# MAdrid1011/transplat

Hardware: AMD Instinct MI355X
Metric: novel views/sec at 256x256, 2 ctx views; PSNR parity vs reference (higher is better)
Workload: dtype fp32 (bf16x3 dense, >= TF32) + bf16x3 attention + fp32 raster; 1 GPU; e2e TranSplat test_step: 1 scene(s) x (2 ctx -> 3 tgt) 256x256; dense mode bf16x3 (split-bf16 products, fp32 accumulation; >= TF32), window-attention mode bf16x3; parallelism=scene-shard x1

## Files before the change

include/transplat_hip.h:

```cpp
#ifndef TRANSPLAT_HIP_H
#define TRANSPLAT_HIP_H

#include <stddef.h>
#include <stdint.h>

#ifdef __cplusplus
extern "C" {
#endif

#define TSPLAT_OK 0
#define TSPLAT_EINVAL (-1)
#define TSPLAT_EHIP (-2)

int tsplat_version(void);

int tsplat_set_debug(int32_t on);

int tsplat_prof_enable(int32_t kernel_id);
int tsplat_prof_read(double* total_ms, int32_t* launches);

typedef struct tsplat_raster_desc {
    int32_t num_gaussians;
    int32_t num_views;
    int32_t views_per_scene;
    int32_t height;
    int32_t width;
    int32_t sh_coeffs;
    int32_t sh_degree;
    int32_t capacity;
} tsplat_raster_desc;

size_t tsplat_raster_workspace_bytes(int32_t num_gaussians, int32_t num_views, int32_t height,
                                     int32_t width, int32_t capacity);

size_t tsplat_raster_num_rendered_offset(int32_t num_gaussians, int32_t num_views, int32_t height,
                                         int32_t width);

int tsplat_raster_fwd(const tsplat_raster_desc* desc,
                      const float* means, const float* cov, const float* shs,
                      const float* opacity, const float* viewmat, const float* projmat,
                      const float* campos, const float* tanfov, const float* bg,
                      const float* scene_scale,
                      float* out_color, int32_t* out_radii,
                      void* workspace, int32_t* status, void* stream);

int tsplat_raster_depth_fwd(const tsplat_raster_desc* desc,
                            const float* means, const float* cov, const float* shs,
                            const float* opacity, const float* viewmat, const float* projmat,
                            const float* campos, const float* tanfov, const float* bg,
                            const float* scene_scale, const float* near, const float* far,
                            int32_t depth_mode,
                            float* out_color, float* out_depth, float* out_alpha,
                            int32_t* out_radii, void* workspace, int32_t* status, void* stream);

size_t tsplat_raster_bwd_workspace_bytes(int32_t num_gaussians, int32_t num_views);

int tsplat_raster_bwd(const tsplat_raster_desc* desc,
                      const float* means, const float* cov, const float* shs,
                      const float* opacity, const float* viewmat, const float* projmat,
                      const float* campos, const float* tanfov, const float* bg,
                      const float* scene_scale,
                      const float* out_color, const float* grad_color, const int32_t* radii,
                      void* fwd_workspace, void* bwd_workspace,
                      float* grad_means, float* grad_cov, float* grad_shs, float* grad_opacity,
                      void* stream);

int tsplat_raster_depth_bwd(const tsplat_raster_desc* desc,
                            const float* means, const float* cov, const float* shs,
                            const float* opacity, const float* viewmat, const float* projmat,
                            const float* campos, const float* tanfov, const float* bg,
                            const float* scene_scale, const float* near, const float* far,
                            int32_t depth_mode,
                            const float* out_color, const float* out_depth, const float* out_alpha,
                            const float* grad_color, const float* grad_depth,
                            const float* grad_alpha, const int32_t* radii,
                            void* fwd_workspace, void* bwd_workspace,
                            float* grad_means, float* grad_cov, float* grad_shs, float* grad_opacity,
                            void* stream);


int tsplat_depth_softmax_fwd(const float* logits, const float* disp, float* coarse, float* pdf_max, int32_t n,
                             int32_t depths, int32_t hw, void* stream);

int tsplat_depth_tail_fwd(const float* fullres, const float* head, const float* near, const float* far, float* depth,
                          float* density, int32_t batch, int32_t views, int32_t hw, void* stream);

int tsplat_raster_cameras(const float* extrinsics, const float* intrinsics, const float* near, const float* far,
                          const float* bg, int32_t bg_per_view, int32_t scale_invariant, int32_t num_views,
                          float* viewmat, float* projmat, float* campos, float* tanfov, float* bg_out, float* scale,
                          void* stream);


int tsplat_uv_coarse_fwd(const float* feat, const float* cams, const float* disp, float* out,
                         int32_t batch, int32_t height, int32_t width, int32_t channels,
                         int32_t depths, void* stream);

int tsplat_uv_cross_fwd(const float* value, const float* key, const float* cams,
                        const float* disp, const float* offsets, const float* logits, float* out,
                        int32_t batch, int32_t height, int32_t width, int32_t channels,
                        int32_t depths, int32_t points, void* stream);

int tsplat_uv_cross_table_fwd(const float* table, const float* cams, const float* disp, const float* offsets,
                              const float* logits, float* out, int32_t batch, int32_t height, int32_t width,
                              int32_t channels, int32_t depths, int32_t points, void* stream);

size_t tsplat_uv_cross_pack_bytes(int32_t batch, int32_t height, int32_t width);
int tsplat_uv_cross_pack_fwd(const float* value, void* packed, int32_t batch, int32_t height, int32_t width,
                             int32_t channels, void* stream);
int tsplat_uv_cross_fused_fwd(const void* packed, const float* key, const float* cams, const float* disp,
                              const float* offsets, const float* logits, float* out, int32_t batch,
                              int32_t height, int32_t width, int32_t channels, int32_t depths, int32_t points,
                              void* stream);
int tsplat_uv_cross_pack_ld_fwd(const float* value, int32_t ld_value, void* packed, int32_t batch, int32_t height,
                                int32_t width, int32_t channels, void* stream);
int tsplat_uv_cross_fused_ld_fwd(const void* packed, const float* key, const float* cams, const float* disp,
                                 const float* offsets, int32_t ld_offsets, const float* logits, int32_t ld_logits,
                                 float* out, int32_t batch, int32_t height, int32_t width, int32_t channels,
                                 int32_t depths, int32_t points, void* stream);

int tsplat_msda_fwd(const float* value, const float* loc, const float* weights, float* out,
                    int32_t n, int32_t height, int32_t width, int32_t channels, int32_t queries,
                    int32_t points, void* stream);

int tsplat_msda_raw_fwd(const float* value, const float* ow, float* out, int32_t n, int32_t height, int32_t width,
                        int32_t channels, int32_t points, int32_t ow_stride, void* stream);

int tsplat_ms_deform_attn_fwd(const float* value, const int64_t* spatial_shapes, const int64_t* level_start_index,
                              const float* sampling_loc, const float* attn_weight, float* out, int32_t batch,
                              int32_t num_keys, int32_t num_heads, int32_t head_dim, int32_t num_levels,
                              int32_t num_queries, int32_t num_points, int32_t im2col_step, void* stream);

int tsplat_sh_rotation_fwd(const float* rotations, const double* basis, float* out, int32_t num_cameras,
                           int32_t d_sh, void* stream);

size_t tsplat_group_norm_workspace_bytes(int32_t n, int32_t c, int64_t hw, int32_t groups);
int tsplat_group_norm_fwd(const float* x, const float* pre_bias, const float* gamma, const float* beta,
                          const float* residual,
                          float* y, void* workspace, int32_t n, int32_t c, int64_t hw, int32_t groups,
                          float eps, int32_t act, void* stream);
int tsplat_group_norm_cat_res_fwd(const float* x, const float* pre_bias, const float* gamma, const float* beta,
                                  const float* residual, const float* residual2, int32_t c1, float* y,
                                  void* workspace, int32_t n, int32_t c, int64_t hw, int32_t groups, float eps,
                                  int32_t act, void* stream);
int tsplat_group_norm_bf16_fwd(const void* x, const float* pre_bias, const float* gamma, const float* beta,
                               const void* residual, void* y, void* workspace, int32_t n, int32_t c, int64_t hw,
                               int32_t groups, float eps, int32_t act, void* stream);

int tsplat_bias_act_fwd(const float* x, const float* bias, const float* residual, float* y, int32_t n, int32_t c,
                        int64_t hw, int32_t act, void* stream);

int tsplat_bias_act_nhwc_fwd(const float* x, const float* bias, const float* res1, const float* res2, float* y,
                             int64_t rows, int32_t c, int32_t act, void* stream);

int tsplat_residual_ln_fwd(const float* x, const float* y, const float* ls, const float* ln_w, const float* ln_b,
                           float ln_eps, float* x_out, float* n_out, int32_t rows, int32_t dim, void* stream);
int tsplat_layer_norm128_fwd(const void* y, int32_t y_bf16, const float* residual, const float* ln_w,
                             const float* ln_b, float ln_eps, void* out, int32_t out_bf16, int32_t rows,
                             void* stream);
int tsplat_residual_ln_bf16_fwd(const float* x, const void* y, const float* ls, const float* ln_w, const float* ln_b,
                                float ln_eps, float* x_out, void* n_out, int32_t rows, int32_t dim, void* stream);

int tsplat_gaussian_adapter_fwd(const float* raw, const float* depths, const float* densities,
                                const float* cams, const float* sh_rot, float* means, float* cov,
                                float* harmonics, float* opacities, int32_t batch, int32_t views,
                                int32_t height, int32_t width, int32_t raw_ch, int32_t d_sh,
                                float scale_min, float scale_max, float opacity_exponent,
                                int32_t gaussians_per_pixel, int32_t raw_nchw, void* stream);

size_t tsplat_win_attn_workspace_bytes(int32_t batch, int32_t height, int32_t width, int32_t key_views,
                                       int32_t splits);
int tsplat_win_attn_fwd(const float* q, const float* k, const float* v, float* out, void* workspace,
                        int32_t batch, int32_t height, int32_t width, int32_t channels,
                        int32_t key_views, int32_t splits, int32_t with_shift, void* stream);

int32_t tsplat_win_attn_split(int32_t batch, int32_t height, int32_t width, int32_t key_views, int32_t splits);
int tsplat_win_attn_partials_fwd(const float* q, const float* k, const float* v, void* workspace, int32_t batch,
                                 int32_t height, int32_t width, int32_t channels, int32_t key_views,
                                 int32_t splits, int32_t with_shift, int32_t key_batch_shift, void* stream);

int tsplat_split_kv_bf16x3(const float* k, const float* v, void* kv_x3, int64_t n, void* stream);
int tsplat_linear_f32_split_x3_fwd(const float* x1, int32_t k1, const float* w, float* out, void* kv_x3, int32_t M,
                                   int32_t N, int32_t x3_from, int32_t flags, void* stream);
int tsplat_win_attn_x3_fwd(const float* q, const void* kv_x3, float* out, void* workspace, int32_t batch,
                           int32_t height, int32_t width, int32_t channels, int32_t key_views, int32_t splits,
                           int32_t with_shift, void* stream);
int tsplat_win_attn_x3_partials_fwd(const float* q, const void* kv_x3, void* workspace, int32_t batch, int32_t height,
                                    int32_t width, int32_t channels, int32_t key_views, int32_t splits,
                                    int32_t with_shift, int32_t key_batch_shift, void* stream);

size_t tsplat_win_attn_bf16_workspace_bytes(int32_t batch, int32_t height, int32_t width, int32_t key_views,
                                            int32_t splits);
int tsplat_win_attn_bf16_fwd(const void* q, const void* k, const void* v, void* out, void* workspace,
                             int32_t batch, int32_t height, int32_t width, int32_t channels,
                             int32_t key_views, int32_t splits, int32_t with_shift, void* stream);
int tsplat_win_attn_bf16_shift_fwd(const void* q, const void* k, const void* v, void* out, void* workspace,
                                   int32_t batch, int32_t height, int32_t width, int32_t channels,
                                   int32_t key_views, int32_t splits, int32_t with_shift,
                                   int32_t key_batch_shift, void* stream);

int tsplat_linear_f32_fwd(const float* x1, int32_t k1, const float* x2, int32_t k2, const float* w,
                          const float* bias, const float* ln_gamma, const float* ln_beta, float ln_eps,
                          const float* residual, float* out, int64_t split_stride, int32_t M, int32_t N,
                          int32_t flags, void* stream);

int tsplat_linear_f32_attn_merge_fwd(const float* partials, int32_t batch, int32_t height, int32_t width,
                                     int32_t key_views, int32_t splits, int32_t with_shift, const float* w,
                                     const float* ln_gamma, const float* ln_beta, float ln_eps,
                                     const float* residual, float* out, int32_t N, int32_t flags, void* stream);

int tsplat_small_inverse(const float* in, float* out, int32_t n, int32_t dim, void* stream);

int tsplat_pack_cameras_fwd(const float* intr, const float* pose, float* cams, int32_t n, void* stream);

int tsplat_cam_gate_fwd(const float* cam, const float* w1, const float* b1, const float* w2, const float* b2,
                        const float* w3, const float* b3, const float* w4, const float* b4, float* gate,
                        int32_t views, int32_t in_features, int32_t channels, void* stream);

int tsplat_mha_f32_fwd(const float* qkv, float* out, int32_t batch, int32_t tokens, int32_t heads,
                       int32_t head_dim, float scale, void* stream);
int tsplat_mha_bias_f32_fwd(const float* qkv, const float* bias, float* out, int32_t batch, int32_t tokens,
                            int32_t heads, int32_t head_dim, float scale, void* stream);
int tsplat_mha_x3_presplit_fwd(const void* qkv_hi, const void* qkv_lo, float* out, int32_t batch, int32_t tokens,
                               int32_t heads, int32_t head_dim, float scale, void* stream);
size_t tsplat_mha_x3_workspace_bytes(int32_t batch, int32_t tokens, int32_t heads, int32_t head_dim);
int tsplat_mha_x3_fwd(const float* qkv, const float* bias, float* out, void* workspace, int32_t batch,
                      int32_t tokens, int32_t heads, int32_t head_dim, float scale, void* stream);

int tsplat_qkv_attention_cf_fwd(const float* qkv, float* out, int32_t batch, int32_t heads, int32_t views,
                                int32_t tokens_per_view, int32_t head_dim, float scale, void* stream);

int tsplat_conv2d_f32_fwd(const float* x1, int32_t c1, const float* x2, int32_t c2, const float* w_packed,
                          const float* bias, float* y, int32_t batch, int32_t height, int32_t width, int32_t c_out,
                          int32_t ksize, int32_t stride, int32_t upsample, int32_t ksplit, void* stream);

int tsplat_conv2d_f32_zsplit_fwd(const float* x1, int32_t c1, const float* x2, int32_t c2, const float* w_packed,
                                 const float* bias, float* y, int32_t batch, int32_t height, int32_t width,
                                 int32_t c_out, int32_t ksize, int32_t stride, int32_t upsample, int32_t ksplit,
                                 int32_t zsplit, float* partials, int32_t* counters, void* stream);

int tsplat_conv2d_bf16x3_fwd(const float* x1, int32_t c1, const float* x2, int32_t c2, const void* w_packed,
                             const float* bias, float* y, int32_t batch, int32_t height, int32_t width,
                             int32_t c_out, int32_t ksize, int32_t stride, int32_t upsample, int32_t ksplit,
                             int32_t zsplit, float* partials, int32_t* counters, void* stream);
int tsplat_conv1x1_bf16x3_scaled_fwd(const float* x, int32_t c_in, const float* scale, const void* w_packed,
                                     const float* bias, float* y, int32_t batch, int32_t height, int32_t width,
                                     int32_t c_out, int32_t channel_last, int32_t ksplit, int32_t zsplit,
                                     float* partials, int32_t* counters, void* stream);

size_t tsplat_wino_weight_floats(int32_t c_out, int32_t c_in);
int tsplat_wino_weight_f32(const float* weight, float* w_packed, int32_t c_out, int32_t c_in, void* stream);
int tsplat_conv3x3_wino_f32_fwd(const float* x, const float* w_packed, const float* bias, float* y, int32_t batch,
                                int32_t c_in, int32_t height, int32_t width, int32_t c_out, int32_t act,
                                void* stream);
int tsplat_conv3x3_wino_cat_f32_fwd(const float* const* srcs, const int32_t* chans, int32_t n_src,
                                    const float* w_packed, const float* bias, float* y, int32_t batch,
                                    int32_t height, int32_t width, int32_t c_out, int32_t act, void* stream);

size_t tsplat_wino_weight_bf16x3_bytes(int32_t c_out, int32_t c_in);
int tsplat_wino_weight_bf16x3(const float* weight, void* w_packed, int32_t c_out, int32_t c_in, void* stream);
int tsplat_conv3x3_wino_bf16x3_fwd(const float* x, const void* w_packed, const float* bias, float* y, int32_t batch,
                                   int32_t c_in, int32_t height, int32_t width, int32_t c_out, int32_t act,
                                   void* stream);
int tsplat_conv3x3_wino_bf16x3_cat_fwd(const float* const* srcs, const int32_t* chans, int32_t n_src,
                                       const void* w_packed, const float* bias, float* y, int32_t batch,
                                       int32_t height, int32_t width, int32_t c_out, int32_t act, void* stream);
int tsplat_conv3x3_wino_bf16x3_ex_fwd(const float* const* srcs, const int32_t* chans, int32_t n_src,
                                      const void* w_packed, const float* bias, const float* residual,
                                      const float* residual2, float* y, int32_t batch, int32_t height, int32_t width,
                                      int32_t c_out, int32_t act, int32_t relu_in, void* stream);

int32_t tsplat_conv3x3_few_form(int32_t batch, int32_t c_in, int32_t height, int32_t width, int32_t c_out);
int tsplat_conv3x3_few_bf16x3_fwd(const float* const* srcs, const int32_t* chans, int32_t n_src,
                                  const void* w_packed, const float* bias, const float* residual,
                                  const float* residual2, float* y, int32_t batch, int32_t height, int32_t width,
                                  int32_t c_out, int32_t act, int32_t relu_in, void* stream);

int tsplat_split_bf16x3(const float* x, void* out, int64_t rows, int32_t k, int32_t weight_order, void* stream);

size_t tsplat_conv2d_bf16_weight_bytes(int32_t c_out, int32_t c_in, int32_t ksize);
int tsplat_conv2d_bf16_fwd(const void* const* srcs, const int32_t* src_channels, int32_t n_src, const int32_t* src_f32,
                           const void* w_packed, const float* bias, void* y, int32_t batch, int32_t height,
                           int32_t width, int32_t c_out, int32_t ksize, int32_t upsample, int32_t act,
                           void* stream);

int tsplat_conv2d_f32_nhwc_fwd(const float* x, int32_t c_in, const float* w_packed, const float* bias,
                               const float* residual, float* y, int32_t batch, int32_t height, int32_t width,
                               int32_t c_out, int32_t ksize, int32_t relu_in, int32_t ksplit, void* stream);

int tsplat_upsample_bilinear_act_fwd(const float* x, const float* bias, float* y, int32_t n, int32_t c,
                                     int32_t height, int32_t width, int32_t scale, int32_t act, void* stream);

int tsplat_resize_bilinear_nhwc_fwd(const float* x, float* y, int32_t n, int32_t height, int32_t width, int32_t c,
                                    int32_t out_height, int32_t out_width, void* stream);

int tsplat_resize_bilinear_nchw_fwd(const float* x, float* y, int32_t planes, int32_t height, int32_t width,
                                    int32_t out_height, int32_t out_width, void* stream);

size_t tsplat_gemm_x3_pack_bytes(int32_t n, int32_t k);
int tsplat_gemm_x3_pack(const float* w, void* wp, int32_t n, int32_t k, void* stream);
int tsplat_gemm_x3_fwd(const float* x, const void* wp, const float* bias, float* out, int32_t m, int32_t n, int32_t k,
                       int32_t ksplit, int32_t act, void* stream);
int tsplat_gemm_x3_cat_fwd(const float* x1, int32_t k1, const float* x2, int32_t k2, const void* wp, const float* bias,
                           float* out, int32_t m, int32_t n, int32_t ksplit, int32_t act, void* stream);

int tsplat_residual_ln_slabs_fwd(const float* x, const float* y, int32_t nslab, const float* ls, const float* ln_w,
                                 const float* ln_b, float ln_eps, float* x_out, float* n_out, int32_t rows,
                                 int32_t dim, void* stream);
int tsplat_residual_ln_slabs_bcast_fwd(const float* x, int32_t x_rows, const float* y, int32_t nslab, const float* ls,
                                       const float* ln_w, const float* ln_b, float ln_eps, float* x_out, float* n_out,
                                       int32_t rows, int32_t dim, void* stream);

int tsplat_da_patches_fwd(const float* image, const float* mean, const float* stdv, float* out, int32_t nimg,
                          int32_t height, int32_t width, int32_t grid_h, int32_t grid_w, int32_t patch, void* stream);

int32_t tsplat_depth_norm_blocks(int32_t out_height, int32_t out_width);
int tsplat_depth_norm_fwd(const float* x, float* resized, float* partials, float* out, int32_t nimg, int32_t height,
                          int32_t width, int32_t out_height, int32_t out_width, void* stream);

size_t tsplat_ssim_workspace_bytes(int32_t n, int32_t height, int32_t width);
int tsplat_ssim_fwd(const float* gt, const float* pred, float* ssim, void* workspace, int32_t n, int32_t height,
                    int32_t width, void* stream);

int tsplat_lpips_scale_fwd(const float* gt, const float* pred, float* out, int32_t n, int32_t height, int32_t width,
                           void* stream);
int32_t tsplat_lpips_tap_blocks(int32_t channels, int32_t height, int32_t width);
size_t tsplat_lpips_workspace_bytes(int32_t n, int32_t channels, int32_t height, int32_t width);
int tsplat_lpips_tap_fwd(const float* feat, const float* lin, void* partials, float* pooled, int32_t n,
                         int32_t channels, int32_t height, int32_t width, void* stream);
int tsplat_lpips_reduce_fwd(const void* workspace, const int32_t* blocks, const int64_t* pixels, int32_t ntaps,
                            float* out, float* out_layers, int32_t n, void* stream);


int tsplat_trajectory_extrinsics(const float* initial, const float* final_, const float* t, double eps,
                                 int32_t num_pairs, int32_t num_steps, float* out, void* stream);

size_t tsplat_quantile_workspace_bytes(int32_t num_requests);
int tsplat_quantile_f32(const float* x, int64_t n, const double* q, const int32_t* positive_only,
                        int32_t num_requests, double* out, void* workspace, void* stream);

int tsplat_video_frames_fwd(const float* color, const float* depth, const double* quantiles, int32_t frames,
                            int32_t height, int32_t width, uint8_t* out, void* stream);

int tsplat_timestamp(void* buf, int32_t slot, void* stream);

#ifdef __cplusplus
}
#endif

#endif
```

transplat_amd/_lib.py:

```python
from __future__ import annotations

import ctypes
import os
from pathlib import Path

import torch

_LIB_PATH = Path(os.environ.get("TSPLAT_LIB") or Path(__file__).resolve().parent / "libtransplat_hip.so")
_lib = None


class RasterDesc(ctypes.Structure):
    _fields_ = [
        ("num_gaussians", ctypes.c_int32),
        ("num_views", ctypes.c_int32),
        ("views_per_scene", ctypes.c_int32),
        ("height", ctypes.c_int32),
        ("width", ctypes.c_int32),
        ("sh_coeffs", ctypes.c_int32),
        ("sh_degree", ctypes.c_int32),
        ("capacity", ctypes.c_int32),
    ]


_P = ctypes.c_void_p
_I32 = ctypes.c_int32

SIGNATURES = {
    "tsplat_version": (ctypes.c_int, []),
    "tsplat_set_debug": (ctypes.c_int, [_I32]),
    "tsplat_timestamp": (ctypes.c_int, [_P, _I32, _P]),
    "tsplat_prof_enable": (ctypes.c_int, [_I32]),
    "tsplat_prof_read": (ctypes.c_int, [ctypes.POINTER(ctypes.c_double), ctypes.POINTER(_I32)]),
    "tsplat_raster_workspace_bytes": (ctypes.c_size_t, [_I32, _I32, _I32, _I32, _I32]),
    "tsplat_raster_num_rendered_offset": (ctypes.c_size_t, [_I32, _I32, _I32, _I32]),
    "tsplat_raster_fwd": (
        ctypes.c_int,
        [ctypes.POINTER(RasterDesc)] + [_P] * 15,
    ),
    "tsplat_raster_depth_fwd": (
        ctypes.c_int,
        [ctypes.POINTER(RasterDesc)] + [_P] * 12 + [_I32] + [_P] * 7,
    ),
    "tsplat_raster_bwd_workspace_bytes": (ctypes.c_size_t, [_I32, _I32]),
    "tsplat_raster_bwd": (
        ctypes.c_int,
        [ctypes.POINTER(RasterDesc)] + [_P] * 20,
    ),
    "tsplat_raster_depth_bwd": (
        ctypes.c_int,
        [ctypes.POINTER(RasterDesc)] + [_P] * 12 + [_I32] + [_P] * 14,
    ),
    "tsplat_uv_coarse_fwd": (ctypes.c_int, [_P] * 4 + [_I32] * 5 + [_P]),
    "tsplat_uv_cross_fwd": (ctypes.c_int, [_P] * 7 + [_I32] * 6 + [_P]),
    "tsplat_uv_cross_table_fwd": (ctypes.c_int, [_P] * 6 + [_I32] * 6 + [_P]),
    "tsplat_uv_cross_pack_bytes": (ctypes.c_size_t, [_I32] * 3),
    "tsplat_uv_cross_pack_fwd": (ctypes.c_int, [_P, _P] + [_I32] * 4 + [_P]),
    "tsplat_uv_cross_fused_fwd": (ctypes.c_int, [_P] * 7 + [_I32] * 6 + [_P]),
    "tsplat_uv_cross_pack_ld_fwd": (ctypes.c_int, [_P, _I32, _P] + [_I32] * 4 + [_P]),
    "tsplat_uv_cross_fused_ld_fwd": (ctypes.c_int, [_P] * 5 + [_I32, _P, _I32, _P] + [_I32] * 6 + [_P]),
    "tsplat_msda_fwd": (ctypes.c_int, [_P] * 4 + [_I32] * 6 + [_P]),
    "tsplat_msda_raw_fwd": (ctypes.c_int, [_P, _P, _P] + [_I32] * 6 + [_P]),
    "tsplat_ms_deform_attn_fwd": (ctypes.c_int, [_P] * 6 + [_I32] * 8 + [_P]),
    "tsplat_win_attn_workspace_bytes": (ctypes.c_size_t, [_I32] * 5),
    "tsplat_win_attn_fwd": (ctypes.c_int, [_P] * 5 + [_I32] * 7 + [_P]),
    "tsplat_win_attn_bf16_workspace_bytes": (ctypes.c_size_t, [_I32] * 5),
    "tsplat_win_attn_bf16_fwd": (ctypes.c_int, [_P] * 5 + [_I32] * 7 + [_P]),
    "tsplat_win_attn_bf16_shift_fwd": (ctypes.c_int, [_P] * 5 + [_I32] * 8 + [_P]),
    "tsplat_group_norm_workspace_bytes": (ctypes.c_size_t, [_I32, _I32, ctypes.c_int64, _I32]),
    "tsplat_group_norm_fwd": (ctypes.c_int, [_P] * 7 + [_I32, _I32, ctypes.c_int64, _I32, ctypes.c_float, _I32, _P]),
    "tsplat_group_norm_cat_res_fwd": (ctypes.c_int, [_P] * 6 + [_I32, _P, _P, _I32, _I32, ctypes.c_int64, _I32,
                                                                ctypes.c_float, _I32, _P]),
    "tsplat_layer_norm128_fwd": (ctypes.c_int, [_P, _I32, _P, _P, _P, ctypes.c_float, _P, _I32, _I32, _P]),
    "tsplat_group_norm_bf16_fwd": (ctypes.c_int, [_P] * 7 + [_I32, _I32, ctypes.c_int64, _I32, ctypes.c_float, _I32,
                                                            _P]),
    "tsplat_sh_rotation_fwd": (ctypes.c_int, [_P] * 3 + [_I32] * 2 + [_P]),
    "tsplat_gaussian_adapter_fwd": (ctypes.c_int, [_P] * 9 + [_I32] * 6 + [ctypes.c_float] * 3 + [_I32, _I32, _P]),
    "tsplat_win_attn_split": (_I32, [_I32] * 5),
    "tsplat_depth_softmax_fwd": (ctypes.c_int, [_P] * 4 + [_I32] * 3 + [_P]),
    "tsplat_depth_tail_fwd": (ctypes.c_int, [_P] * 6 + [_I32] * 3 + [_P]),
    "tsplat_ssim_workspace_bytes": (ctypes.c_size_t, [_I32] * 3),
    "tsplat_ssim_fwd": (ctypes.c_int, [_P] * 4 + [_I32] * 3 + [_P]),
    "tsplat_lpips_scale_fwd": (ctypes.c_int, [_P] * 3 + [_I32] * 3 + [_P]),
    "tsplat_lpips_tap_blocks": (_I32, [_I32] * 3),
    "tsplat_lpips_workspace_bytes": (ctypes.c_size_t, [_I32] * 4),
    "tsplat_lpips_tap_fwd": (ctypes.c_int, [_P] * 4 + [_I32] * 4 + [_P]),
    "tsplat_lpips_reduce_fwd": (ctypes.c_int, [_P, _P, _P, _I32, _P, _P, _I32, _P]),
    "tsplat_raster_cameras": (ctypes.c_int, [_P] * 5 + [_I32] * 3 + [_P] * 7),
    "tsplat_small_inverse": (ctypes.c_int, [_P, _P, _I32, _I32, _P]),
    "tsplat_trajectory_extrinsics": (ctypes.c_int, [_P, _P, _P, ctypes.c_double, _I32, _I32, _P, _P]),
    "tsplat_quantile_workspace_bytes": (ctypes.c_size_t, [_I32]),
    "tsplat_quantile_f32": (ctypes.c_int, [_P, ctypes.c_int64, ctypes.POINTER(ctypes.c_double),
                                           ctypes.POINTER(_I32), _I32, _P, _P, _P]),
    "tsplat_video_frames_fwd": (ctypes.c_int, [_P, _P, _P, _I32, _I32, _I32, _P, _P]),
    "tsplat_pack_cameras_fwd": (ctypes.c_int, [_P, _P, _P, _I32, _P]),
    "tsplat_cam_gate_fwd": (ctypes.c_int, [_P] * 10 + [_I32] * 3 + [_P]),
    "tsplat_mha_f32_fwd": (ctypes.c_int, [_P, _P, _I32, _I32, _I32, _I32, ctypes.c_float, _P]),
    "tsplat_mha_bias_f32_fwd": (ctypes.c_int, [_P, _P, _P, _I32, _I32, _I32, _I32, ctypes.c_float, _P]),
    "tsplat_mha_x3_workspace_bytes": (ctypes.c_size_t, [_I32] * 4),
    "tsplat_mha_x3_fwd": (ctypes.c_int, [_P, _P, _P, _P, _I32, _I32, _I32, _I32, ctypes.c_float, _P]),
    "tsplat_mha_x3_presplit_fwd": (ctypes.c_int, [_P, _P, _P, _I32, _I32, _I32, _I32, ctypes.c_float, _P]),
    "tsplat_qkv_attention_cf_fwd": (ctypes.c_int, [_P, _P] + [_I32] * 5 + [ctypes.c_float, _P]),
    "tsplat_conv2d_f32_fwd": (ctypes.c_int, [_P, _I32, _P, _I32, _P, _P, _P] + [_I32] * 8 + [_P]),
    "tsplat_conv2d_f32_zsplit_fwd": (ctypes.c_int, [_P, _I32, _P, _I32, _P, _P, _P] + [_I32] * 9 + [_P, _P, _P]),
    "tsplat_conv2d_bf16x3_fwd": (ctypes.c_int, [_P, _I32, _P, _I32, _P, _P, _P] + [_I32] * 9 + [_P, _P, _P]),
    "tsplat_conv1x1_bf16x3_scaled_fwd": (ctypes.c_int, [_P, _I32, _P, _P, _P, _P] + [_I32] * 7 + [_P, _P, _P]),
    "tsplat_resize_bilinear_nhwc_fwd": (ctypes.c_int, [_P, _P] + [_I32] * 6 + [_P]),
    "tsplat_resize_bilinear_nchw_fwd": (ctypes.c_int, [_P, _P] + [_I32] * 5 + [_P]),
    "tsplat_upsample_bilinear_act_fwd": (ctypes.c_int, [_P, _P, _P] + [_I32] * 6 + [_P]),
    "tsplat_conv2d_f32_nhwc_fwd": (ctypes.c_int, [_P, _I32, _P, _P, _P, _P] + [_I32] * 7 + [_P]),
    "tsplat_residual_ln_fwd": (ctypes.c_int, [_P] * 5 + [ctypes.c_float, _P, _P, _I32, _I32, _P]),
    "tsplat_residual_ln_slabs_fwd": (ctypes.c_int, [_P, _P, _I32, _P, _P, _P, ctypes.c_float, _P, _P, _I32, _I32, _P]),
    "tsplat_gemm_x3_pack_bytes": (ctypes.c_size_t, [_I32, _I32]),
    "tsplat_gemm_x3_pack": (ctypes.c_int, [_P, _P, _I32, _I32, _P]),
    "tsplat_gemm_x3_fwd": (ctypes.c_int, [_P, _P, _P, _P, _I32, _I32, _I32, _I32, _I32, _P]),
    "tsplat_gemm_x3_cat_fwd": (ctypes.c_int, [_P, _I32, _P, _I32, _P, _P, _P] + [_I32] * 4 + [_P]),
    "tsplat_residual_ln_slabs_bcast_fwd": (ctypes.c_int, [_P, _I32, _P, _I32, _P, _P, _P, ctypes.c_float, _P, _P, _I32,
                                                          _I32, _P]),
    "tsplat_da_patches_fwd": (ctypes.c_int, [_P] * 4 + [_I32] * 6 + [_P]),
    "tsplat_depth_norm_blocks": (_I32, [_I32, _I32]),
    "tsplat_depth_norm_fwd": (ctypes.c_int, [_P] * 4 + [_I32] * 5 + [_P]),
    "tsplat_residual_ln_bf16_fwd": (ctypes.c_int, [_P] * 5 + [ctypes.c_float, _P, _P, _I32, _I32, _P]),
    "tsplat_bias_act_fwd": (ctypes.c_int, [_P] * 4 + [_I32, _I32, ctypes.c_int64, _I32, _P]),
    "tsplat_bias_act_nhwc_fwd": (ctypes.c_int, [_P, _P, _P, _P, _P, ctypes.c_int64, _I32, _I32, _P]),
    "tsplat_win_attn_partials_fwd": (ctypes.c_int, [_P] * 4 + [_I32] * 8 + [_P]),
    "tsplat_split_kv_bf16x3": (ctypes.c_int, [_P, _P, _P, ctypes.c_int64, _P]),
    "tsplat_linear_f32_split_x3_fwd": (ctypes.c_int, [_P, _I32, _P, _P, _P] + [_I32] * 4 + [_P]),
    "tsplat_win_attn_x3_fwd": (ctypes.c_int, [_P] * 4 + [_I32] * 7 + [_P]),
    "tsplat_win_attn_x3_partials_fwd": (ctypes.c_int, [_P] * 3 + [_I32] * 8 + [_P]),
    "tsplat_linear_f32_attn_merge_fwd": (ctypes.c_int, [_P] + [_I32] * 6 + [_P] * 3 + [ctypes.c_float, _P, _P, _I32,
                                                                                       _I32, _P]),
    "tsplat_linear_f32_fwd": (ctypes.c_int, [_P, _I32, _P, _I32] + [_P] * 4 + [ctypes.c_float, _P, _P, ctypes.c_int64]
                              + [_I32] * 3 + [_P]),
    "tsplat_wino_weight_floats": (ctypes.c_size_t, [_I32, _I32]),
    "tsplat_wino_weight_f32": (ctypes.c_int, [_P, _P, _I32, _I32, _P]),
    "tsplat_conv3x3_wino_f32_fwd": (ctypes.c_int, [_P, _P, _P, _P] + [_I32] * 6 + [_P]),
    "tsplat_conv3x3_wino_cat_f32_fwd": (ctypes.c_int, [_P, _P, _I32, _P, _P, _P] + [_I32] * 5 + [_P]),
    "tsplat_wino_weight_bf16x3_bytes": (ctypes.c_size_t, [_I32, _I32]),
    "tsplat_wino_weight_bf16x3": (ctypes.c_int, [_P, _P, _I32, _I32, _P]),
    "tsplat_conv3x3_wino_bf16x3_fwd": (ctypes.c_int, [_P, _P, _P, _P] + [_I32] * 6 + [_P]),
    "tsplat_conv3x3_wino_bf16x3_cat_fwd": (ctypes.c_int, [_P, _P, _I32, _P, _P, _P] + [_I32] * 5 + [_P]),
    "tsplat_conv3x3_wino_bf16x3_ex_fwd": (ctypes.c_int, [_P, _P, _I32, _P, _P, _P, _P, _P] + [_I32] * 6 + [_P]),
    "tsplat_conv3x3_few_form": (ctypes.c_int32, [_I32] * 5),
    "tsplat_conv3x3_few_bf16x3_fwd": (ctypes.c_int, [_P, _P, _I32, _P, _P, _P, _P, _P] + [_I32] * 6 + [_P]),
    "tsplat_split_bf16x3": (ctypes.c_int, [_P, _P, ctypes.c_int64, _I32, _I32, _P]),
    "tsplat_conv2d_bf16_weight_bytes": (ctypes.c_size_t, [_I32, _I32, _I32]),
    "tsplat_conv2d_bf16_fwd": (ctypes.c_int, [_P, _P, _I32, _P, _P, _P, _P] + [_I32] * 7 + [_P]),
}

ERRORS = {-1: "invalid argument", -2: "HIP launch error"}


def lib_path() -> Path:
    return _LIB_PATH


def load(build_if_missing: bool = False):
    global _lib
    if _lib is not None:
        return _lib
    if not _LIB_PATH.exists():
        if build_if_missing:
            from .build import build

            build()
        else:
            raise RuntimeError(
                f"transplat HIP library not built ({_LIB_PATH}); run `python -m transplat_amd.build`"
            )
    lib = ctypes.CDLL(str(_LIB_PATH), mode=os.RTLD_NOW | os.RTLD_GLOBAL)
    for name, (res, args) in SIGNATURES.items():
        fn = getattr(lib, name)
        fn.restype = res
        fn.argtypes = args
    if os.environ.get("TSPLAT_DEBUG", "0") == "1":
        lib.tsplat_set_debug(1)
    _lib = lib
    return lib


def debug_enabled() -> bool:
    lib = load()
    was = lib.tsplat_set_debug(1)
    lib.tsplat_set_debug(was)
    return bool(was)


ROUTE_HOOK = None


def check(status: int, what: str, route: str | None = None) -> None:
    if status != 0:
        raise RuntimeError(f"{what} failed: {ERRORS.get(status, status)}")
    if ROUTE_HOOK is not None:
        ROUTE_HOOK(what, route)


def ptr(t: torch.Tensor | None) -> int | None:
    if t is None:
        return None
    if not t.is_cuda:
        raise RuntimeError("transplat HIP ops need device tensors (no CPU path)")
    return t.data_ptr()


def stream_ptr(device: torch.device | None = None) -> int:
    return torch.cuda.current_stream(device).cuda_stream


PROF_IDS = {"raster_preprocess": 1, "raster_scan": 2, "raster_scatter": 3, "raster_render": 4,
            "uv_coarse": 5, "uv_cross": 6, "msda": 7, "win_attn": 8, "raster": 9,
            "group_norm": 10, "uv_cross_table": 11, "linear": 12, "mha": 13, "conv": 14, "wino_conv": 15,
            "gemm_x3": 16, "raster_bwd_render": 17, "raster_bwd_preprocess": 18, "raster_bwd": 19}


def prof_enable(name: str | None) -> None:
    check(load().tsplat_prof_enable(PROF_IDS[name] if name else 0), "tsplat_prof_enable")


def prof_read() -> tuple[float, int]:
    ms = ctypes.c_double(0.0)
    n = _I32(0)
    check(load().tsplat_prof_read(ctypes.byref(ms), ctypes.byref(n)), "tsplat_prof_read")
    return ms.value, n.value
```

transplat_amd/csrc/conv.hip:

```cpp
#include "common.h"
#include "mfma.h"
#include "prof.h"

namespace tsplat {
namespace conv {

constexpr int kMaxWaves = 16;

struct Args {
    const float* x1;
    const float* x2;
    const float* wp;
    const float* bias;
    const float* res;
    const float* scale;
    int cl_out;
    float* y;
    float* part;
    int* cnt;
    int zsplit;
    int c1, c2, cout, n;
    int hin, win;
    int hv, wv;
    int hout, wout;
    int npx;
};

template <bool NHWC>
__device__ __forceinline__ void tile_epilogue(const Args& p, const floatx16& acc, float* sred) {
    const int lane = threadIdx.x & 63, w = threadIdx.x >> 6, ksplit = blockDim.x >> 6;
    const int cot = blockIdx.y;
    const int hwo = p.hout * p.wout;
#pragma unroll
    for (int r = 0; r < 16; ++r) sred[(w * 16 + r) * 64 + lane] = acc[r];
    __syncthreads();
    const int tile = blockIdx.x + gridDim.x * blockIdx.y;
    if (p.zsplit > 1) {
        typedef __attribute__((address_space(1))) unsigned gu32;
        unsigned* mine = reinterpret_cast<unsigned*>(p.part + ((size_t)tile * p.zsplit + blockIdx.z) * 1024);
        for (int idx = threadIdx.x; idx < 1024; idx += blockDim.x) {
            float s = 0.f;
            for (int k = 0; k < ksplit; ++k) s += sred[(k * 16 + (idx >> 6)) * 64 + (idx & 63)];
            __hip_atomic_store((gu32*)(mine + idx), __float_as_uint(s), __ATOMIC_RELAXED, __HIP_MEMORY_SCOPE_AGENT);
        }
        asm volatile("s_waitcnt vmcnt(0)" ::: "memory");
        __syncthreads();
        int* flag = reinterpret_cast<int*>(sred + ksplit * 1024);
        if (threadIdx.x == 0) {
            const int t = __hip_atomic_fetch_add(p.cnt + tile, 1, __ATOMIC_RELEASE, __HIP_MEMORY_SCOPE_AGENT);
            const bool last = t == p.zsplit - 1;
            if (last) {
                __builtin_amdgcn_fence(__ATOMIC_ACQUIRE, "agent");
                asm volatile("s_waitcnt vmcnt(0)" ::: "memory");
                __hip_atomic_store(p.cnt + tile, 0, __ATOMIC_RELAXED, __HIP_MEMORY_SCOPE_AGENT);
            }
            *flag = last;
        }
        __syncthreads();
        if (!*flag) return;
        const float* all = p.part + (size_t)tile * p.zsplit * 1024;
        for (int idx = threadIdx.x; idx < 1024; idx += blockDim.x) {
            float s = 0.f;
            for (int z = 0; z < p.zsplit; ++z) s += all[(size_t)z * 1024 + idx];
            sred[idx] = s;
        }
        __syncthreads();
    }
    const int nsum = p.zsplit > 1 ? 1 : ksplit;
    for (int idx = threadIdx.x; idx < 1024; idx += blockDim.x) {
        int r, l;
        if (NHWC) {
            const int col = idx & 31, pl = idx >> 5;
            r = ((col >> 3) << 2) | (col & 3);
            l = ((col >> 2) & 1) * 32 + pl;
        } else {
            r = idx >> 6;
            l = idx & 63;
        }
        float s = 0.f;
        for (int k = 0; k < nsum; ++k) s += sred[(k * 16 + r) * 64 + l];
        const int co = cot * 32 + 8 * (r >> 2) + 4 * (l >> 5) + (r & 3);
        const int q = blockIdx.x * 32 + (l & 31);
        if (co >= p.cout || q >= p.npx) continue;
        if (p.bias) s += p.bias[co];
        size_t o;
        if (NHWC) {
            o = (size_t)q * p.cout + co;
        } else {
            const int qn = q / hwo, qp = q - qn * hwo;
            o = ((size_t)qn * p.cout + co) * hwo + qp;
        }
        if (p.res) s += p.res[o];
        p.y[o] = s;
    }
}

template <int KS, int S, int UP, int G, bool NHWC, bool RELU>
__global__ void __launch_bounds__(1024) conv_f32_kernel(Args p) {
    extern __shared__ float sred[];
    constexpr int T = KS * KS, PAD = KS / 2;
    constexpr int B = G * T;
    const int lane = threadIdx.x & 63, w = threadIdx.x >> 6, ksplit = blockDim.x >> 6;
    const int c = lane & 31, h = lane >> 5;
    const int cot = blockIdx.y;
    const int hwo = p.hout * p.wout, hwi = p.hin * p.win;
    const int px = blockIdx.x * 32 + c;
    const int pxc = min(px, p.npx - 1);
    const int nb = pxc / hwo, pix = pxc - nb * hwo;
    const int oy = pix / p.wout, ox = pix - oy * p.wout;
    const int cp_all = (p.c1 + p.c2) >> 1, cp1 = p.c1 >> 1;

    int off[T];
    unsigned vmask = 0;
#pragma unroll
    for (int t = 0; t < T; ++t) {
        const int ky = t / KS, kx = t - ky * KS;
        const int iy = oy * S + ky - PAD, ix = ox * S + kx - PAD;
        const bool v = px < p.npx && iy >= 0 && iy < p.hv && ix >= 0 && ix < p.wv;
        if (NHWC)
            off[t] = v ? (nb * hwi + iy * p.win + ix) * p.c1 : 0;
        else
            off[t] = v ? (UP ? (iy >> 1) * p.win + (ix >> 1) : iy * p.win + ix) : 0;
        vmask |= (unsigned)v << t;
    }
    const size_t wtap = (size_t)cp_all * 64;
    const float* wbase = p.wp + (size_t)cot * T * wtap + lane;
    auto chan = [&](int cp) -> const float* {
        if (NHWC) return p.x1 + 2 * cp + h;
        return cp < cp1 ? p.x1 + ((size_t)nb * p.c1 + 2 * cp + h) * hwi
                        : p.x2 + ((size_t)nb * p.c2 + 2 * (cp - cp1) + h) * hwi;
    };
    const int gw = blockIdx.z * ksplit + w, gstride = ksplit * p.zsplit;
    const int ncp = cp_all > gw ? (cp_all - gw + gstride - 1) / gstride : 0;
    const int nbatch = (ncp + G - 1) / G;
    auto load = [&](int bi, float* a, float* b) {
#pragma unroll
        for (int g = 0; g < G; ++g) {
            const int i = bi * G + g;
            const bool ok = i < ncp;
            const int cp = gw + min(i, ncp - 1) * gstride;
            const float* src = chan(cp);
            const float* wq = wbase + (size_t)cp * 64;
#pragma unroll
            for (int t = 0; t < T; ++t) {
                const float av = wq[t * wtap];
                const float bv = RELU ? fmaxf(src[off[t]], 0.f) : src[off[t]];
                const unsigned ma = ok ? ~0u : 0u;
                const unsigned mb = (ok && ((vmask >> t) & 1)) ? ~0u : 0u;
                a[g * T + t] = __uint_as_float(__float_as_uint(av) & ma);
                b[g * T + t] = __uint_as_float(__float_as_uint(bv) & mb);
            }
        }
    };

    floatx16 acc;
#pragma unroll
    for (int r = 0; r < 16; ++r) acc[r] = 0.f;
    if constexpr (KS == 3) {
        const int nb = G == 4 ? min(nbatch, 1) : nbatch;
#pragma unroll 1
        for (int bi = 0; bi < nb; ++bi) {
            float ca[B], cb[B];
            load(bi, ca, cb);
            __builtin_amdgcn_sched_barrier(0);
#pragma unroll
            for (int k = 0; k < B; ++k) acc = __builtin_amdgcn_mfma_f32_32x32x2f32(ca[k], cb[k], acc, 0, 0, 0);
        }
    } else {
        float ca[B], cb[B], na[B], nbv[B];
        if (nbatch > 0) load(0, ca, cb);
        __builtin_amdgcn_sched_barrier(0);
#pragma unroll 1
        for (int bi = 0; bi < nbatch; ++bi) {
            const bool more = bi + 1 < nbatch;
            if (more) load(bi + 1, na, nbv);
            __builtin_amdgcn_sched_barrier(0);
#pragma unroll
            for (int k = 0; k < B; ++k) acc = __builtin_amdgcn_mfma_f32_32x32x2f32(ca[k], cb[k], acc, 0, 0, 0);
            if (more) {
#pragma unroll
                for (int k = 0; k < B; ++k) {
                    ca[k] = na[k];
                    cb[k] = nbv[k];
                }
            }
        }
    }

    tile_epilogue<NHWC>(p, acc, sred);
}

template <int KS, int S, int UP, int NB, bool SC = false>
__global__ void __launch_bounds__(1024) conv_x3_kernel(Args p) {
    extern __shared__ float sred[];
    constexpr int T = KS * KS, PAD = KS / 2;
    const int lane = threadIdx.x & 63, w = threadIdx.x >> 6, ksplit = blockDim.x >> 6;
    const int h = lane >> 5;
    const int cot = blockIdx.y;
    const int hwo = p.hout * p.wout, hwi = p.hin * p.win;
    const int px = blockIdx.x * 32 + (lane & 31);
    const int pxc = min(px, p.npx - 1);
    const int nb = pxc / hwo, pix = pxc - nb * hwo;
    const int oy = pix / p.wout, ox = pix - oy * p.wout;
    const int ci = p.c1 + p.c2, ng = (ci + 15) >> 4;
    int off[T];
    unsigned vmask = 0;
#pragma unroll
    for (int t = 0; t < T; ++t) {
        const int ky = t / KS, kx = t - ky * KS;
        const int iy = oy * S + ky - PAD, ix = ox * S + kx - PAD;
        const bool v = px < p.npx && iy >= 0 && iy < p.hv && ix >= 0 && ix < p.wv;
        off[t] = v ? (UP ? (iy >> 1) * p.win + (ix >> 1) : iy * p.win + ix) : 0;
        vmask |= (unsigned)v << t;
    }
    const uint4* wbase = reinterpret_cast<const uint4*>(p.wp) + (size_t)cot * T * ng * 128 + lane;
    const int units = ng * T;
    const int gw = blockIdx.z * ksplit + w, gstride = ksplit * p.zsplit;
    const int nu = units > gw ? (units - gw + gstride - 1) / gstride : 0;
    const float* x1 = p.x1 + (size_t)nb * p.c1 * hwi;
    const float* x2 = p.x2 ? p.x2 + (size_t)nb * p.c2 * hwi : p.x1;
    const float* sc = SC && p.scale ? p.scale + (size_t)nb * ci : nullptr;

    floatx16 acc;
#pragma unroll
    for (int r = 0; r < 16; ++r) acc[r] = 0.f;
#pragma unroll 1
    for (int b0 = 0; b0 < nu; b0 += NB) {
        float xv[NB][8];
        uint4 ah[NB], al[NB];
#pragma unroll
        for (int k = 0; k < NB; ++k) {
            const int i = b0 + k;
            const bool ok = i < nu;
            const int u = gw + min(i, nu - 1) * gstride;
            const int g = u / T, t = u - g * T;
            const uint4* wq = wbase + (size_t)(t * ng + g) * 128;
            const unsigned ma = ok ? ~0u : 0u;
            const uint4 a0 = wq[0], a1 = wq[64];
            ah[k] = make_uint4(a0.x & ma, a0.y & ma, a0.z & ma, a0.w & ma);
            al[k] = make_uint4(a1.x & ma, a1.y & ma, a1.z & ma, a1.w & ma);
            int o = 0;
            bool tv = false;
#pragma unroll
            for (int tt = 0; tt < T; ++tt)
                if (tt == t) {
                    o = off[tt];
                    tv = (vmask >> tt) & 1;
                }
#pragma unroll
            for (int j = 0; j < 8; ++j) {
                const int ch = 16 * g + 8 * h + j;
                const int cc = min(ch, ci - 1);
                const float* src = cc < p.c1 ? x1 + (size_t)cc * hwi : x2 + (size_t)(cc - p.c1) * hwi;
                float v = src[o];
                if (SC && sc) v *= sc[cc];
                const unsigned mb = (ok && tv && ch < ci) ? ~0u : 0u;
                xv[k][j] = __uint_as_float(__float_as_uint(v) & mb);
            }
        }
        __builtin_amdgcn_sched_barrier(0);
#pragma unroll
        for (int k = 0; k < NB; ++k) {
            uint32_t hi[4], lo[4];
#pragma unroll
            for (int q = 0; q < 4; ++q) split_pair(xv[k][2 * q], xv[k][2 * q + 1], hi[q], lo[q]);
            const bf16x8 bh = __builtin_bit_cast(bf16x8, make_uint4(hi[0], hi[1], hi[2], hi[3]));
            const bf16x8 bl = __builtin_bit_cast(bf16x8, make_uint4(lo[0], lo[1], lo[2], lo[3]));
            const bf16x8 wh = __builtin_bit_cast(bf16x8, ah[k]), wl = __builtin_bit_cast(bf16x8, al[k]);
            acc = __builtin_amdgcn_mfma_f32_32x32x16_bf16(wl, bh, acc, 0, 0, 0);
            acc = __builtin_amdgcn_mfma_f32_32x32x16_bf16(wh, bl, acc, 0, 0, 0);
            acc = __builtin_amdgcn_mfma_f32_32x32x16_bf16(wh, bh, acc, 0, 0, 0);
        }
    }
    if constexpr (SC) {
        if (p.cl_out) {
            tile_epilogue<true>(p, acc, sred);
            return;
        }
    }
    tile_epilogue<false>(p, acc, sred);
}

}
}

extern "C" int tsplat_conv2d_f32_zsplit_fwd(const float* x1, int32_t c1, const float* x2, int32_t c2,
                                            const float* w_packed, const float* bias, float* y, int32_t batch,
                                            int32_t height, int32_t width, int32_t c_out, int32_t ksize,
                                            int32_t stride, int32_t upsample, int32_t ksplit, int32_t zsplit,
                                            float* partials, int32_t* counters, void* stream_) {
    using namespace tsplat::conv;
    if (!x1 || !w_packed || !y || batch <= 0 || height <= 0 || width <= 0 || c_out <= 0) return TSPLAT_EINVAL;
    if (zsplit < 1 || zsplit > 64 || (zsplit > 1 && (!partials || !counters))) return TSPLAT_EINVAL;
    if (c1 <= 0 || (c1 & 1) || c2 < 0 || (c2 & 1) || (c2 > 0 && !x2)) return TSPLAT_EINVAL;
    if (!(ksize == 1 || ksize == 3) || !(stride == 1 || stride == 2) || !(upsample == 0 || upsample == 1))
        return TSPLAT_EINVAL;
    if (ksplit < 1 || ksplit > kMaxWaves) return TSPLAT_EINVAL;
    Args p{};
    p.zsplit = zsplit;
    p.part = partials;
    p.cnt = counters;
    p.x1 = x1;
    p.x2 = x2;
    p.wp = w_packed;
    p.bias = bias;
    p.y = y;
    p.c1 = c1;
    p.c2 = c2;
    p.cout = c_out;
    p.n = batch;
    p.hin = height;
    p.win = width;
    p.hv = upsample ? 2 * height : height;
    p.wv = upsample ? 2 * width : width;
    const int pad = ksize / 2;
    p.hout = (p.hv + 2 * pad - ksize) / stride + 1;
    p.wout = (p.wv + 2 * pad - ksize) / stride + 1;
    if (p.hout <= 0 || p.wout <= 0) return TSPLAT_EINVAL;
    const int64_t npx = (int64_t)batch * p.hout * p.wout;
    const int64_t in_elems = (int64_t)batch * (c1 > c2 ? c1 : c2) * height * width;
    if (npx >= (1ll << 31) || in_elems >= (1ll << 31)) return TSPLAT_EINVAL;
    p.npx = (int)npx;
    hipStream_t stream = (hipStream_t)stream_;
    const dim3 grid((unsigned)((npx + 31) / 32), (unsigned)((c_out + 31) / 32), (unsigned)zsplit);
    const dim3 block(64 * ksplit);
    const size_t lds = (size_t)ksplit * 16 * 64 * sizeof(float) + 16;
    TSPLAT_PROF_BEGIN(tsplat::prof::kConv, stream);
#define TSPLAT_CONV_LAUNCH(KS, S, UP, G) \
    hipLaunchKernelGGL((conv_f32_kernel<KS, S, UP, G, false, false>), grid, block, lds, stream, p)
    const int per_wave = ((c1 + c2) / 2 + ksplit * zsplit - 1) / (ksplit * zsplit);
    const bool wide = per_wave >= (ksize == 3 ? 2 : 16);
    const bool one = ksize == 3 && per_wave >= 3 && per_wave <= 4;
    if (ksize == 3 && stride == 1 && !upsample) {
        if (one) TSPLAT_CONV_LAUNCH(3, 1, 0, 4); else if (wide) TSPLAT_CONV_LAUNCH(3, 1, 0, 2); else TSPLAT_CONV_LAUNCH(3, 1, 0, 1);
    } else if (ksize == 3 && stride == 2 && !upsample) {
        if (one) TSPLAT_CONV_LAUNCH(3, 2, 0, 4); else if (wide) TSPLAT_CONV_LAUNCH(3, 2, 0, 2); else TSPLAT_CONV_LAUNCH(3, 2, 0, 1);
    } else if (ksize == 3 && stride == 1 && upsample) {
        if (one) TSPLAT_CONV_LAUNCH(3, 1, 1, 4); else if (wide) TSPLAT_CONV_LAUNCH(3, 1, 1, 2); else TSPLAT_CONV_LAUNCH(3, 1, 1, 1);
    } else if (ksize == 1 && stride == 1 && !upsample) {
        if (wide) TSPLAT_CONV_LAUNCH(1, 1, 0, 16); else TSPLAT_CONV_LAUNCH(1, 1, 0, 8);
    } else if (ksize == 1 && stride == 2 && !upsample) {
        TSPLAT_CONV_LAUNCH(1, 2, 0, 8);
    } else {
        return TSPLAT_EINVAL;
    }
#undef TSPLAT_CONV_LAUNCH
    TSPLAT_PROF_END(tsplat::prof::kConv, stream);
    TSPLAT_CHECK_LAUNCH();
    return TSPLAT_OK;
}

extern "C" int tsplat_conv2d_f32_fwd(const float* x1, int32_t c1, const float* x2, int32_t c2, const float* w_packed,
                                     const float* bias, float* y, int32_t batch, int32_t height, int32_t width,
                                     int32_t c_out, int32_t ksize, int32_t stride, int32_t upsample, int32_t ksplit,
                                     void* stream_) {
    return tsplat_conv2d_f32_zsplit_fwd(x1, c1, x2, c2, w_packed, bias, y, batch, height, width, c_out, ksize, stride,
                                        upsample, ksplit, 1, nullptr, nullptr, stream_);
}

extern "C" int tsplat_conv2d_f32_nhwc_fwd(const float* x, int32_t c_in, const float* w_packed, const float* bias,
                                          const float* residual, float* y, int32_t batch, int32_t height,
                                          int32_t width, int32_t c_out, int32_t ksize, int32_t relu_in,
                                          int32_t ksplit, void* stream_) {
    using namespace tsplat::conv;
    if (!x || !w_packed || !y || batch <= 0 || height <= 0 || width <= 0 || c_out <= 0) return TSPLAT_EINVAL;
    if (c_in <= 0 || (c_in & 1) || !(ksize == 1 || ksize == 3) || ksplit < 1 || ksplit > kMaxWaves)
        return TSPLAT_EINVAL;
    const int64_t elems = (int64_t)batch * height * width * (c_in > c_out ? c_in : c_out);
    if (elems >= (1ll << 31)) return TSPLAT_EINVAL;
    Args p{};
    p.x1 = x;
    p.wp = w_packed;
    p.bias = bias;
    p.res = residual;
    p.y = y;
    p.c1 = c_in;
    p.cout = c_out;
    p.n = batch;
    p.hin = p.hv = p.hout = height;
    p.win = p.wv = p.wout = width;
    p.npx = batch * height * width;
    p.zsplit = 1;
    hipStream_t stream = (hipStream_t)stream_;
    const dim3 grid((unsigned)((p.npx + 31) / 32), (unsigned)((c_out + 31) / 32));
    const dim3 block(64 * ksplit);
    const size_t lds = (size_t)ksplit * 16 * 64 * sizeof(float);
    const int per_wave = (c_in / 2 + ksplit - 1) / ksplit;
    const bool wide = per_wave >= (ksize == 3 ? 2 : 16);
    TSPLAT_PROF_BEGIN(tsplat::prof::kConv, stream);
#define TSPLAT_CONV_LAUNCH(KS, G, RELU) \
    hipLaunchKernelGGL((conv_f32_kernel<KS, 1, 0, G, true, RELU>), grid, block, lds, stream, p)
    if (ksize == 3) {
        if (relu_in) {
            if (wide) TSPLAT_CONV_LAUNCH(3, 2, true); else TSPLAT_CONV_LAUNCH(3, 1, true);
        } else {
            if (wide) TSPLAT_CONV_LAUNCH(3, 2, false); else TSPLAT_CONV_LAUNCH(3, 1, false);
        }
    } else {
        if (relu_in) {
            if (wide) TSPLAT_CONV_LAUNCH(1, 16, true); else TSPLAT_CONV_LAUNCH(1, 8, true);
        } else {
            if (wide) TSPLAT_CONV_LAUNCH(1, 16, false); else TSPLAT_CONV_LAUNCH(1, 8, false);
        }
    }
#undef TSPLAT_CONV_LAUNCH
    TSPLAT_PROF_END(tsplat::prof::kConv, stream);
    TSPLAT_CHECK_LAUNCH();
    return TSPLAT_OK;
}

static int conv_x3_launch(const float* x1, int32_t c1, const float* x2, int32_t c2, const void* w_packed,
                          const float* bias, float* y, int32_t batch, int32_t height, int32_t width, int32_t c_out,
                          int32_t ksize, int32_t stride, int32_t upsample, int32_t ksplit, int32_t zsplit,
                          float* partials, int32_t* counters, bool scaled, const float* scale, int32_t cl_out,
                          void* stream_) {
    using namespace tsplat::conv;
    if (!x1 || !w_packed || !y || batch <= 0 || height <= 0 || width <= 0 || c_out <= 0) return TSPLAT_EINVAL;
    if (zsplit < 1 || zsplit > 64 || (zsplit > 1 && (!partials || !counters))) return TSPLAT_EINVAL;
    if (c1 <= 0 || c2 < 0 || (c2 > 0 && !x2)) return TSPLAT_EINVAL;
    if (!(ksize == 1 || ksize == 3) || !(stride == 1 || stride == 2) || !(upsample == 0 || upsample == 1) ||
        (upsample && stride != 1))
        return TSPLAT_EINVAL;
    if (ksplit < 1 || ksplit > kMaxWaves) return TSPLAT_EINVAL;
    Args p{};
    p.zsplit = zsplit;
    p.part = partials;
    p.cnt = counters;
    p.x1 = x1;
    p.x2 = c2 > 0 ? x2 : nullptr;
    p.wp = (const float*)w_packed;
    p.bias = bias;
    p.y = y;
    p.scale = scale;
    p.cl_out = cl_out;
    p.c1 = c1;
    p.c2 = c2;
    p.cout = c_out;
    p.n = batch;
    p.hin = height;
    p.win = width;
    p.hv = upsample ? 2 * height : height;
    p.wv = upsample ? 2 * width : width;
    const int pad = ksize / 2;
    p.hout = (p.hv + 2 * pad - ksize) / stride + 1;
    p.wout = (p.wv + 2 * pad - ksize) / stride + 1;
    if (p.hout <= 0 || p.wout <= 0) return TSPLAT_EINVAL;
    const int64_t npx = (int64_t)batch * p.hout * p.wout;
    const int64_t in_elems = (int64_t)batch * (c1 > c2 ? c1 : c2) * height * width;
    if (npx >= (1ll << 31) || in_elems >= (1ll << 31)) return TSPLAT_EINVAL;
    p.npx = (int)npx;
    hipStream_t stream = (hipStream_t)stream_;
    const dim3 grid((unsigned)((npx + 31) / 32), (unsigned)((c_out + 31) / 32), (unsigned)zsplit);
    const dim3 block(64 * ksplit);
    const size_t lds = (size_t)ksplit * 16 * 64 * sizeof(float) + 16;
    const int units = (c1 + c2 + 15) / 16 * ksize * ksize;
    const int per_wave = (units + ksplit * zsplit - 1) / (ksplit * zsplit);
    const int nb = per_wave <= 4 ? per_wave : 2;
    TSPLAT_PROF_BEGIN(tsplat::prof::kConv, stream);
#define TSPLAT_X3_LAUNCH(KS, S, UP)                                                                       \
    do {                                                                                                  \
        if (nb == 1) hipLaunchKernelGGL((conv_x3_kernel<KS, S, UP, 1>), grid, block, lds, stream, p);     \
        else if (nb == 3) hipLaunchKernelGGL((conv_x3_kernel<KS, S, UP, 3>), grid, block, lds, stream, p); \
        else if (nb == 4) hipLaunchKernelGGL((conv_x3_kernel<KS, S, UP, 4>), grid, block, lds, stream, p); \
        else hipLaunchKernelGGL((conv_x3_kernel<KS, S, UP, 2>), grid, block, lds, stream, p);             \
    } while (0)
    if (scaled) {
        if (nb == 1) hipLaunchKernelGGL((conv_x3_kernel<1, 1, 0, 1, true>), grid, block, lds, stream, p);
        else if (nb == 3) hipLaunchKernelGGL((conv_x3_kernel<1, 1, 0, 3, true>), grid, block, lds, stream, p);
        else if (nb == 4) hipLaunchKernelGGL((conv_x3_kernel<1, 1, 0, 4, true>), grid, block, lds, stream, p);
        else hipLaunchKernelGGL((conv_x3_kernel<1, 1, 0, 2, true>), grid, block, lds, stream, p);
    } else if (ksize == 3 && stride == 1 && !upsample) TSPLAT_X3_LAUNCH(3, 1, 0);
    else if (ksize == 3 && stride == 2) TSPLAT_X3_LAUNCH(3, 2, 0);
    else if (ksize == 3) TSPLAT_X3_LAUNCH(3, 1, 1);
    else if (stride == 1) TSPLAT_X3_LAUNCH(1, 1, 0);
    else TSPLAT_X3_LAUNCH(1, 2, 0);
#undef TSPLAT_X3_LAUNCH
    TSPLAT_PROF_END(tsplat::prof::kConv, stream);
    TSPLAT_CHECK_LAUNCH();
    return TSPLAT_OK;
}

extern "C" int tsplat_conv2d_bf16x3_fwd(const float* x1, int32_t c1, const float* x2, int32_t c2,
                                        const void* w_packed, const float* bias, float* y, int32_t batch,
                                        int32_t height, int32_t width, int32_t c_out, int32_t ksize, int32_t stride,
                                        int32_t upsample, int32_t ksplit, int32_t zsplit, float* partials,
                                        int32_t* counters, void* stream_) {
    return conv_x3_launch(x1, c1, x2, c2, w_packed, bias, y, batch, height, width, c_out, ksize, stride, upsample,
                          ksplit, zsplit, partials, counters, false, nullptr, 0, stream_);
}

extern "C" int tsplat_conv1x1_bf16x3_scaled_fwd(const float* x, int32_t c_in, const float* scale, const void* w_packed,
                                                const float* bias, float* y, int32_t batch, int32_t height,
                                                int32_t width, int32_t c_out, int32_t channel_last, int32_t ksplit,
                                                int32_t zsplit, float* partials, int32_t* counters, void* stream_) {
    if (channel_last != 0 && channel_last != 1) return TSPLAT_EINVAL;
    return conv_x3_launch(x, c_in, nullptr, 0, w_packed, bias, y, batch, height, width, c_out, 1, 1, 0, ksplit, zsplit,
                          partials, counters, true, scale, channel_last, stream_);
}
```

transplat_amd/kernels.py:

```python
from __future__ import annotations

import ctypes
import functools
import os
import weakref
from collections import namedtuple

import torch
import torch.nn.functional as F

from . import _lib


def _f32(t: torch.Tensor) -> torch.Tensor:
    if t.dtype != torch.float32:
        t = t.float()
    return t.contiguous()


_DERIVED: dict = {}
_DERIVED_MAX = 512


def _derived(tensor, tag: str, make):
# ... 575 lines not shown
    rc = lib.tsplat_layer_norm128_fwd(_lib.ptr(yc), int(yc.dtype == torch.bfloat16), _lib.ptr(res),
                                      _lib.ptr(_f32(norm.weight)), _lib.ptr(_f32(norm.bias)), float(norm.eps),
                                      _lib.ptr(out), int(out_dtype == torch.bfloat16), yc.numel() // 128,
                                      _lib.stream_ptr(y.device))
    _lib.check(rc, "tsplat_layer_norm128_fwd", "bf16 I/O, fp32 statistics" if yc.dtype == torch.bfloat16 else "fp32")
    return out


def depth_softmax(logits, disp):
    lib = _lib.load()
    n, d, h, w = logits.shape
    lf = _f32(logits)
    df = _f32(disp.reshape(n, d))
    coarse = torch.empty((n, 1, h, w), dtype=torch.float32, device=logits.device)
    pmax = torch.empty_like(coarse)
    _lib.check(lib.tsplat_depth_softmax_fwd(_lib.ptr(lf), _lib.ptr(df), _lib.ptr(coarse), _lib.ptr(pmax), n, d,
                                            h * w, _lib.stream_ptr(logits.device)), "tsplat_depth_softmax_fwd")
    return coarse, pmax


def depth_tail(fullres, head, near, far):
    lib = _lib.load()
    b, v = near.shape
    hw = fullres.shape[-2] * fullres.shape[-1]
    fr, hd, nr, fa = _f32(fullres), _f32(head), _f32(near), _f32(far)
    depth = torch.empty((b, v, hw), dtype=torch.float32, device=fullres.device)
    dens = torch.empty_like(depth)
    _lib.check(lib.tsplat_depth_tail_fwd(_lib.ptr(fr), _lib.ptr(hd), _lib.ptr(nr), _lib.ptr(fa), _lib.ptr(depth),
                                         _lib.ptr(dens), b, v, hw, _lib.stream_ptr(fullres.device)),
               "tsplat_depth_tail_fwd")
    return depth, dens


def ssim(gt, pred):
    lib = _lib.load()
    if not (gt.is_cuda and pred.is_cuda):
        raise RuntimeError("transplat HIP ops need device tensors (no CPU path)")
    if gt.shape != pred.shape:
        raise ValueError(f"ssim: ground truth {tuple(gt.shape)} != prediction {tuple(pred.shape)}")
    if gt.dim() != 4 or gt.shape[1] != 3:
        raise ValueError(f"ssim: expected [n, 3, H, W] images, got {tuple(gt.shape)}")
    n, _, h, w = gt.shape
    if h < 11 or w < 11:
        raise ValueError(f"ssim: the 11 x 11 window does not fit a {h} x {w} image")
    out = torch.empty((n,), dtype=torch.float32, device=gt.device)
    if n == 0:
        return out
    g, p = _f32(gt), _f32(pred)
    ws = torch.empty(int(lib.tsplat_ssim_workspace_bytes(n, h, w)), dtype=torch.uint8, device=gt.device)
    _lib.check(lib.tsplat_ssim_fwd(_lib.ptr(g), _lib.ptr(p), _lib.ptr(out), _lib.ptr(ws), n, h, w,
                                   _lib.stream_ptr(gt.device)), "tsplat_ssim_fwd")
    return out


LPIPS_CHUNK = 8


def lpips_scale(gt, pred):
    lib = _lib.load()
    n, _, h, w = gt.shape
    out = torch.empty((2 * n, 3, h, w), dtype=torch.float32, device=gt.device)
    _lib.check(lib.tsplat_lpips_scale_fwd(_lib.ptr(gt), _lib.ptr(pred), _lib.ptr(out), n, h, w,
                                          _lib.stream_ptr(gt.device)), "tsplat_lpips_scale_fwd")
    return out


def _lpips_tap_into(feat, lin, partials, pool: bool):
    lib = _lib.load()
    n2, c, h, w = feat.shape
    pooled = torch.empty((n2, c, h // 2, w // 2), dtype=torch.float32, device=feat.device) if pool else None
    _lib.check(lib.tsplat_lpips_tap_fwd(_lib.ptr(feat), _lib.ptr(lin), _lib.ptr(partials), _lib.ptr(pooled), n2 // 2, c,
                                        h, w, _lib.stream_ptr(feat.device)), "tsplat_lpips_tap_fwd")
    return pooled


def _lpips_reduce(workspace, n: int, blocks, pixels, out, layers):
    lib = _lib.load()
    pix = ctypes.cast((ctypes.c_int64 * len(pixels))(*pixels), ctypes.c_void_p)
    _lib.check(lib.tsplat_lpips_reduce_fwd(_lib.ptr(workspace), _int32_array(blocks), pix, len(blocks), _lib.ptr(out),
                                           _lib.ptr(layers), n, _lib.stream_ptr(workspace.device)),
               "tsplat_lpips_reduce_fwd")


def lpips_tap(feat, lin, pool: bool = True):
    lib = _lib.load()
    if not (feat.is_cuda and lin.is_cuda):
        raise RuntimeError("transplat HIP ops need device tensors (no CPU path)")
    if feat.dim() != 4 or feat.shape[0] % 2 or feat.shape[0] == 0 or tuple(lin.shape) != (feat.shape[1],):
        raise ValueError(f"lpips_tap: features {tuple(feat.shape)} and weights {tuple(lin.shape)}")
    f, v = _f32(feat), _f32(lin)
    n2, c, h, w = f.shape
    n = n2 // 2
    blocks = int(lib.tsplat_lpips_tap_blocks(c, h, w))
    ws = torch.empty(int(lib.tsplat_lpips_workspace_bytes(n, c, h, w)) // 8, dtype=torch.float64, device=f.device)
    pooled = _lpips_tap_into(f, v, ws, pool)
    out = torch.empty((n,), dtype=torch.float32, device=f.device)
    _lpips_reduce(ws, n, [blocks], [h * w], out, None)
    return out, pooled


def lpips(gt, pred, net, return_layers: bool = False):
    from .evaluation.lpips_vgg import MIN_SIZE, VGG_BLOCKS

    lib = _lib.load()
    if not (gt.is_cuda and pred.is_cuda):
        raise RuntimeError("transplat HIP ops need device tensors (no CPU path)")
    if gt.shape != pred.shape:
        raise ValueError(f"lpips: ground truth {tuple(gt.shape)} != prediction {tuple(pred.shape)}")
    if gt.dim() != 4 or gt.shape[1] != 3:
        raise ValueError(f"lpips: expected [n, 3, H, W] images, got {tuple(gt.shape)}")
    n, _, h, w = gt.shape
    if h < MIN_SIZE or w < MIN_SIZE:
        raise ValueError(f"lpips: a {h} x {w} image leaves the fifth VGG block an empty map (H, W >= {MIN_SIZE})")
    if net.device != gt.device:
        raise RuntimeError(f"lpips: weights on {net.device}, images on {gt.device} (use LpipsVGG.to)")
    out = torch.empty((n,), dtype=torch.float32, device=gt.device)
    layers = torch.empty((n, len(VGG_BLOCKS)), dtype=torch.float32, device=gt.device) if return_layers else None
    g, p = _f32(gt), _f32(pred)
    shapes = [(net.lins[k].shape[0], h >> k, w >> k) for k in range(len(VGG_BLOCKS))]
    blocks = [int(lib.tsplat_lpips_tap_blocks(*s)) for s in shapes]
    pixels = [hk * wk for _, hk, wk in shapes]
    for at in range(0, n, LPIPS_CHUNK):
        m = min(LPIPS_CHUNK, n - at)
        ws = torch.empty(m * sum(blocks), dtype=torch.float64, device=gt.device)
        x = lpips_scale(g[at:at + m], p[at:at + m])
        conv, offset = 0, 0
        for k, count in enumerate(VGG_BLOCKS):
            for _ in range(count):
                weight, bias = net.convs[conv]
                x = conv3x3_wino(x, weight, bias, act="relu", precision="fp32")
                conv += 1
            x = _lpips_tap_into(x, net.lins[k], ws[offset:offset + m * blocks[k]], pool=k + 1 < len(VGG_BLOCKS))
            offset += m * blocks[k]
        _lpips_reduce(ws, m, blocks, pixels, out[at:at + m], layers[at:at + m] if return_layers else None)
    return (out, layers) if return_layers else out


_MHA_X3_ROWS = 2048


def mha_x3_ok(rows: int) -> bool:
    return _DENSE == "bf16x3" and rows <= _MHA_X3_ROWS


def mha_presplit(qkv_split, heads: int, scale: float):
    lib = _lib.load()
    _, b, n, c3 = qkv_split.shape
    d = c3 // (3 * heads)
    x = qkv_split.contiguous()
    out = torch.empty((b, n, heads * d), dtype=torch.float32, device=x.device)
    _lib.check(lib.tsplat_mha_x3_presplit_fwd(_lib.ptr(x[0]), _lib.ptr(x[1]), _lib.ptr(out), b, n, heads, d, float(scale),
                                              _lib.stream_ptr(x.device)), "tsplat_mha_x3_presplit_fwd")
    return out


def mha(qkv, heads: int, scale: float, bias=None, precision: str | None = None):
    lib = _lib.load()
    b, n, c3 = qkv.shape
    d = c3 // (3 * heads)
    x = _f32(qkv)
    out = torch.empty((b, n, heads * d), dtype=torch.float32, device=qkv.device)
    if precision is None:
        precision = "bf16x3" if _DENSE == "bf16x3" and b * n <= _MHA_X3_ROWS else "fp32"
    if precision == "bf16x3":
        ws = torch.empty(int(lib.tsplat_mha_x3_workspace_bytes(b, n, heads, d)), dtype=torch.uint8, device=x.device)
        _lib.check(lib.tsplat_mha_x3_fwd(_lib.ptr(x), _lib.ptr(_f32(bias)) if bias is not None else None,
                                         _lib.ptr(out), _lib.ptr(ws), b, n, heads, d, float(scale),
                                         _lib.stream_ptr(qkv.device)), "tsplat_mha_x3_fwd")
        return out
    if bias is not None:
        _lib.check(lib.tsplat_mha_bias_f32_fwd(_lib.ptr(x), _lib.ptr(_f32(bias)), _lib.ptr(out), b, n, heads, d,
                                               float(scale), _lib.stream_ptr(qkv.device)), "tsplat_mha_bias_f32_fwd")
        return out
    _lib.check(lib.tsplat_mha_f32_fwd(_lib.ptr(x), _lib.ptr(out), b, n, heads, d, float(scale),
                                      _lib.stream_ptr(qkv.device)), "tsplat_mha_f32_fwd")
    return out


_CONV_MODE = os.environ.get("TSPLAT_CONV", "auto")
_CONV_MAX_FLOP = 1.5e9
_CONV1_WAVES = 16384
_CONV1_PAIRS = 8
_CONV3_WAVES = 8192
_CONV3_PAIRS = 2
_ZSPLIT = -1
_ZSPLIT_WGS = 256
_ZSPLIT_MIN = 1
_ZSPLIT_CNT: dict = {}
_ZSPLIT_SLAB = 1 << 20


def _zsplit_counters(device, tiles: int):
    if tiles > _ZSPLIT_SLAB // 16:
        raise ValueError(f"zsplit launch of {tiles} tiles exceeds the counter slab's per-launch share")
    slab = _ZSPLIT_CNT.get(device)
    if slab is None:
        slab = [torch.zeros(_ZSPLIT_SLAB, dtype=torch.int32, device=device), 0]
        _ZSPLIT_CNT[device] = slab
    if slab[1] + tiles > _ZSPLIT_SLAB:
        slab[1] = 0
    view = slab[0][slab[1]:slab[1] + tiles]
    slab[1] += tiles
    return view


def _wave_split(tiles: int, work: int, max_waves: int, per_wave: int) -> int:
    ksplit = 16
    while ksplit > 1 and (tiles * ksplit > max_waves or work < per_wave * ksplit):
        ksplit //= 2
    return ksplit


def _zsplit_factor(tiles: int, more) -> int:
    if _ZSPLIT == 0:
        return 1
    z = 1
    while z < 64 and tiles * 2 * z <= _ZSPLIT_WGS and more(z) and (_ZSPLIT < 0 or 2 * z <= _ZSPLIT):
        z *= 2
    return z


def conv_zsplit(tiles: int, pairs: int, ksplit: int, k: int) -> int:
    per_batch = _ZSPLIT_MIN if k == 3 else 4 * _ZSPLIT_MIN
    return _zsplit_factor(tiles, lambda z: -(-pairs // (ksplit * z)) > per_batch)


def _pack_conv(weight):
    co, ci, k = weight.shape[:3]
    cot = (co + 31) // 32
    w = torch.zeros((cot * 32, ci, k * k), dtype=torch.float32, device=weight.device)
    w[:co] = weight.float().reshape(co, ci, k * k)
    return w.reshape(cot, 32, ci // 2, 2, k * k).permute(0, 4, 2, 3, 1).contiguous()


def conv_pack_weight(weight):
    return _derived(weight, "conv", _pack_conv)


def _pack_conv_x3(weight):
    co, ci = weight.shape[:2]
    k = weight.shape[2] if weight.dim() == 4 else 1
    cot, ng = (co + 31) // 32, (ci + 15) // 16
    w = torch.zeros((cot * 32, ng * 16, k * k), dtype=torch.float32, device=weight.device)
    w[:co, :ci] = weight.float().reshape(co, ci, k * k)
    a = w.reshape(cot, 32, ng, 2, 8, k * k).permute(0, 5, 2, 3, 1, 4)
    hi = a.to(torch.bfloat16)
    lo = (a - hi.float()).to(torch.bfloat16)
    return torch.stack((hi, lo), dim=3).contiguous()


def conv_pack_weight_x3(weight):
    return _derived(weight, "conv_x3", _pack_conv_x3)


def conv_x3_wins(npx: int, ci: int, co: int, k: int) -> bool:
    if k == 1:
        return True
    return ci >= 64 and _conv_flop(npx, co, ci, k) >= 0.5e9


def _conv_x3_shape(tiles: int, units: int):
    ksplit = _wave_split(tiles, units, _CONV3_WAVES, 1)
    return ksplit, _zsplit_factor(tiles, lambda z: units >= 2 * ksplit * 2 * z)


def _conv2d_direct_x3(lib, a, b, c1, c2, weight, bias, n, h, w, co, k, stride, upsample, y):
    hout, wout = y.shape[2], y.shape[3]
    tiles = ((n * hout * wout + 31) // 32) * ((co + 31) // 32)
    ksplit, z = _conv_x3_shape(tiles, (c1 + c2 + 15) // 16 * k * k)
    part = cnt = None
    if z > 1:
        part = torch.empty(tiles * z * 1024, dtype=torch.float32, device=y.device)
        cnt = _zsplit_counters(y.device, tiles)
    pb = _f32(bias) if bias is not None else None
    rc = lib.tsplat_conv2d_bf16x3_fwd(_lib.ptr(a), c1, _lib.ptr(b), c2, _lib.ptr(conv_pack_weight_x3(weight)),
                                      _lib.ptr(pb), _lib.ptr(y), n, h, w, co, k, stride, int(upsample), ksplit, z,
                                      _lib.ptr(part), _lib.ptr(cnt), _lib.stream_ptr(y.device))
    _lib.check(rc, "tsplat_conv2d_bf16x3_fwd")
    return y


def conv1x1_scaled(x, scale, weight, bias=None, channel_last: bool = False):
    lib = _lib.load()
    n, ci, h, w = x.shape
    co = weight.shape[0]
    a, sc = _f32(x), _f32(scale)
    if tuple(sc.shape) != (n, ci) or weight.shape[1] != ci:
        raise ValueError(f"scale {tuple(sc.shape)} / weight {tuple(weight.shape)} do not match x {tuple(x.shape)}")
    y = torch.empty((n, h * w, co) if channel_last else (n, co, h, w), dtype=torch.float32, device=x.device)
    tiles = ((n * h * w + 31) // 32) * ((co + 31) // 32)
    ksplit, z = _conv_x3_shape(tiles, (ci + 15) // 16)
    part = cnt = None
    if z > 1:
        part = torch.empty(tiles * z * 1024, dtype=torch.float32, device=y.device)
        cnt = _zsplit_counters(y.device, tiles)
    pb = _f32(bias) if bias is not None else None
    rc = lib.tsplat_conv1x1_bf16x3_scaled_fwd(_lib.ptr(a), ci, _lib.ptr(sc), _lib.ptr(conv_pack_weight_x3(weight)),
                                              _lib.ptr(pb), _lib.ptr(y), n, h, w, co, int(channel_last), ksplit, z,
                                              _lib.ptr(part), _lib.ptr(cnt), _lib.stream_ptr(y.device))
    _lib.check(rc, "tsplat_conv1x1_bf16x3_scaled_fwd")
    return y


def conv2d_direct(x1, weight, bias=None, stride: int = 1, x2=None, upsample: bool = False):
    lib = _lib.load()
    n, c1, h, w = x1.shape
    a = _f32(x1)
    b = _f32(x2) if x2 is not None else None
    c2 = b.shape[1] if b is not None else 0
    if b is not None and (b.shape[0] != n or b.shape[2:] != x1.shape[2:]):
        raise ValueError(f"x2 {tuple(b.shape)} does not match x1 {tuple(x1.shape)}")
    co, ci, k = weight.shape[:3]
    if ci != c1 + c2:
        raise ValueError(f"weight {tuple(weight.shape)} does not match {c1} + {c2} input channels")
    hv, wv = (2 * h, 2 * w) if upsample else (h, w)
    hout, wout = (hv + 2 * (k // 2) - k) // stride + 1, (wv + 2 * (k // 2) - k) // stride + 1
    y = torch.empty((n, co, hout, wout), dtype=torch.float32, device=x1.device)
    if split_mode() and conv_x3_wins(n * hout * wout, c1 + c2, co, k):
        return _conv2d_direct_x3(lib, a, b, c1, c2, weight, bias, n, h, w, co, k, stride, upsample, y)
    tiles = ((n * hout * wout + 31) // 32) * ((co + 31) // 32)
    pairs = ci // 2
    cap, min_pairs = (_CONV3_WAVES, _CONV3_PAIRS) if k == 3 else (_CONV1_WAVES, _CONV1_PAIRS)
    ksplit = _wave_split(tiles, pairs, cap, min_pairs)
    zsplit = conv_zsplit(tiles, pairs, ksplit, k) if ksplit == 16 else 1
    pb = _f32(bias) if bias is not None else None
    part = cnt = None
    if zsplit > 1:
        part = torch.empty(tiles * zsplit * 1024, dtype=torch.float32, device=x1.device)
        cnt = _zsplit_counters(x1.device, tiles)
    rc = lib.tsplat_conv2d_f32_zsplit_fwd(_lib.ptr(a), c1, _lib.ptr(b), c2, _lib.ptr(conv_pack_weight(weight)),
                                          _lib.ptr(pb), _lib.ptr(y), n, h, w, co, k, stride, int(upsample), ksplit,
                                          zsplit, _lib.ptr(part), _lib.ptr(cnt), _lib.stream_ptr(x1.device))
    _lib.check(rc, "tsplat_conv2d_f32_zsplit_fwd")
    return y


_WINO_MODE = os.environ.get("TSPLAT_WINO", "auto")
_WINO_ACT = {"none": 0, "relu": 1, "gelu": 2}


def _pack_wino(weight):
    lib = _lib.load()
    co, ci = weight.shape[:2]
    packed = torch.empty(int(lib.tsplat_wino_weight_floats(co, ci)), dtype=torch.float32, device=weight.device)
    w = _f32(weight)
    _lib.check(lib.tsplat_wino_weight_f32(_lib.ptr(w), _lib.ptr(packed), co, ci, _lib.stream_ptr(weight.device)),
               "tsplat_wino_weight_f32")
    return packed


def wino_pack_weight(weight):
    return _derived(weight, "wino", _pack_wino)


WINO_MAX_CI_PAD = 1024




def conv_unfold_gemm(x, weight, bias, stride: int, padding: int):
    n, ci, h, w = x.shape
    co, _, kh, kw = weight.shape
    ho, wo = (h + 2 * padding - kh) // stride + 1, (w + 2 * padding - kw) // stride + 1
    cols = F.unfold(x, (kh, kw), padding=padding, stride=stride)
    wm = weight.reshape(co, -1)
    y = torch.empty((n, co, ho * wo), dtype=torch.float32, device=x.device)
    with torch.autocast("cuda", enabled=False):
        for i in range(n):
            if bias is not None:
                torch.addmm(bias.view(co, 1), wm, cols[i], out=y[i])
            else:
                torch.mm(wm, cols[i], out=y[i])
    return y.view(n, co, ho, wo)


def conv_transpose_direct(x, weight, bias, s: int):
    ci, co = weight.shape[:2]
    w1 = _derived(weight, "convT", lambda t: t.permute(1, 2, 3, 0).reshape(co * s * s, ci, 1, 1).contiguous())
    b1 = _derived(bias, "convT_b", lambda t: t.repeat_interleave(s * s).contiguous()) if bias is not None else None
    return F.pixel_shuffle(conv2d_direct(x, w1, b1, 1), s)


def conv_transpose_forward(mod, x):
    st = _square(mod.stride)
    if (_square(mod.kernel_size) == st > 0 and _square(mod.padding) == 0 and mod.groups == 1
            and _square(mod.output_padding) == 0 and _square(mod.dilation) == 1 and x.is_cuda
            and x.dtype == torch.float32 and mod.weight.dtype == torch.float32 and x.shape[1] % 2 == 0
            and not torch.is_autocast_enabled("cuda")):
        return conv_transpose_direct(x.contiguous(), mod.weight, mod.bias, st)
    return torch.nn.ConvTranspose2d.forward(mod, x)


def install_conv2d_dispatch(module) -> int:
    n = 0
    for m in module.modules():
        if type(m) is torch.nn.Conv2d:
            m.forward = functools.partial(conv2d_forward, m)
            n += 1
        elif type(m) is torch.nn.ConvTranspose2d:
            m.forward = functools.partial(conv_transpose_forward, m)
            n += 1
    return n


_DENSE = "fp32"
_DENSE_MODES = ("fp32", "bf16x3")


class dense_precision:

    def __init__(self, mode: str):
        if mode not in _DENSE_MODES:
            raise ValueError(f"dense precision {mode!r} not in {_DENSE_MODES}")
        self.mode, self.prev, self.prev_tf32 = mode, None, None

    def __enter__(self):
        global _DENSE
        self.prev, _DENSE = _DENSE, self.mode
        self.prev_tf32 = torch.backends.cuda.matmul.allow_tf32
        torch.backends.cuda.matmul.allow_tf32 = False
        return self

    def __exit__(self, *exc):
        global _DENSE
        _DENSE = self.prev
        torch.backends.cuda.matmul.allow_tf32 = self.prev_tf32
        return False


def split_mode() -> bool:
    return _DENSE == "bf16x3"


_ATTN = "fp32"
ATTN_MODES = ("fp32", "bf16x3", "bf16")


def auto_attention(dense_dtype: str) -> str:
    return dense_dtype if dense_dtype in ("bf16", "bf16x3") else "fp32"


class attention_precision:

    def __init__(self, mode: str):
        if mode not in ATTN_MODES:
            raise ValueError(f"attention precision {mode!r}")
        self.mode, self.prev = mode, None

    def __enter__(self):
        global _ATTN
        self.prev, _ATTN = _ATTN, self.mode
        return self

    def __exit__(self, *exc):
        global _ATTN
        _ATTN = self.prev
        return False


def split_bf16x3(x: torch.Tensor, weight_order: bool = False) -> torch.Tensor:
    lib = _lib.load()
    xf = _f32(x)
    k = xf.shape[-1]
    out = torch.empty((*xf.shape[:-1], 3 * k), dtype=torch.bfloat16, device=xf.device)
    _lib.check(lib.tsplat_split_bf16x3(_lib.ptr(xf), _lib.ptr(out), xf.numel() // k, k, int(weight_order),
                                       _lib.stream_ptr(xf.device)), "tsplat_split_bf16x3")
    return out


def _split_weight(weight):
    return _derived(weight, "split", lambda w: split_bf16x3(w, weight_order=True))


def linear_bf16x3(x, weight, bias=None, act: str = "none", cache: bool = True):
    k, n = x.shape[-1], weight.shape[0]
    w3 = _split_weight(weight) if cache else split_bf16x3(weight, weight_order=True)
    x3 = split_bf16x3(x).reshape(-1, 3 * k)
    with torch.autocast("cuda", enabled=False):
        if bias is not None:
            y = torch.addmm(_f32(bias), x3, w3.t(), out_dtype=torch.float32)
        else:
            y = torch.mm(x3, w3.t(), out_dtype=torch.float32)
    y = y.reshape(*x.shape[:-1], n)
    if act == "gelu":
        y = F.gelu(y)
    return y


_LINX = False


def linear_xf32_ok(x, weight) -> bool:
    if not (_LINX and _DENSE == "bf16x3" and x.is_cuda and x.dtype == torch.float32
            and weight.dtype == torch.float32 and not torch.is_autocast_enabled("cuda")):
        return False
    n, k = weight.shape
    m = x.numel() // max(k, 1)
    return n % 4 == 0 and ((n >= 1024 and m >= 512) or (m >= 4096 and n >= 512))


def linear_xf32(x, weight, bias=None, act: str = "none"):
    prev = torch.backends.cuda.matmul.allow_tf32
    torch.backends.cuda.matmul.allow_tf32 = True
    try:
        y = torch.matmul(x, weight.t())
    finally:
        torch.backends.cuda.matmul.allow_tf32 = prev
    if bias is None and act == "none":
        return y
    y = y.contiguous()
    bb = _f32(bias) if bias is not None else None
    lib = _lib.load()
    rc = lib.tsplat_bias_act_nhwc_fwd(_lib.ptr(y), _lib.ptr(bb), None, None, _lib.ptr(y), y.numel() // y.shape[-1],
                                      y.shape[-1], _ACTS[act], _lib.stream_ptr(y.device))
    _lib.check(rc, "tsplat_bias_act_nhwc_fwd")
    return y


GEMM_LOG = None


def gemm_x3_ok(x, weight) -> bool:
    if not (_DENSE == "bf16x3" and x.is_cuda and x.dtype == torch.float32
            and weight.dtype == torch.float32 and not torch.is_autocast_enabled("cuda")):
        return False
    n = weight.shape[0]
    k = weight.numel() // n
    return k % 4 == 0 and n % 4 == 0 and x.shape[-1] == k


def gemm_x3_takes(x, weight) -> bool:
    return gemm_x3_ok(x, weight) and x.numel() // x.shape[-1] >= 64


def _pack_gemm(weight):
    lib = _lib.load()
    n = weight.shape[0]
    k = weight.numel() // n
    wf = _f32(weight)
    wp = torch.empty(int(lib.tsplat_gemm_x3_pack_bytes(n, k)), dtype=torch.uint8, device=weight.device)
    _lib.check(lib.tsplat_gemm_x3_pack(_lib.ptr(wf), _lib.ptr(wp), n, k, _lib.stream_ptr(weight.device)),
               "tsplat_gemm_x3_pack")
    return wp


def _gemm_pack(weight):
    return _derived(weight, "gemm_x3", _pack_gemm)


def gemm_ksplit(m: int, n: int, k: int) -> int:
    tiles = -(-m // 64) * -(-n // 128)
    nchunk = -(-k // 64)
    s = max(1, min(nchunk // 2, 256 // tiles))
    while s > 1 and (s - 1) * -(-nchunk // s) >= nchunk:
        s -= 1
    return s


_GEMM_CAT = True


def gemm_x3(x, weight, bias=None, act: str = "none", ksplit: int = 1, x2=None):
    lib = _lib.load()
    n = weight.shape[0]
    k = weight.numel() // n
    k1 = x.shape[-1]
    if x2 is not None and not (_GEMM_CAT and k1 % 64 == 0 and x2.shape[:-1] == x.shape[:-1]):
        x, x2 = torch.cat([x, x2], dim=-1), None
    xf = _f32(x)
    x2f = _f32(x2) if x2 is not None else None
    m = xf.numel() // (k1 if x2 is not None else k)
    if ksplit == 0:
        ksplit = 1 if act != "none" else gemm_ksplit(m, n, k)
    if act == "split":
        if ksplit != 1:
            raise ValueError("gemm_x3: the split output needs ksplit 1")
        out = torch.empty((2, *x.shape[:-1], n), dtype=torch.bfloat16, device=x.device)
    else:
        shape = (*x.shape[:-1], n) if ksplit == 1 else (ksplit, *x.shape[:-1], n)
        out = torch.empty(shape, dtype=torch.float32, device=x.device)
    if GEMM_LOG is not None:
        GEMM_LOG.append((m, n, k, ksplit))
    pb = _lib.ptr(_f32(bias)) if bias is not None else None
    acti = {"none": 0, "gelu": 1, "split": 2}[act]
    if x2f is not None:
        rc = lib.tsplat_gemm_x3_cat_fwd(_lib.ptr(xf), k1, _lib.ptr(x2f), k - k1, _lib.ptr(_gemm_pack(weight)), pb,
                                        _lib.ptr(out), m, n, ksplit, acti, _lib.stream_ptr(x.device))
        _lib.check(rc, "tsplat_gemm_x3_cat_fwd", "bf16x3")
        return out
    rc = lib.tsplat_gemm_x3_fwd(_lib.ptr(xf), _lib.ptr(_gemm_pack(weight)), pb, _lib.ptr(out), m, n, k, ksplit, acti,
                                _lib.stream_ptr(x.device))
    _lib.check(rc, "tsplat_gemm_x3_fwd", "bf16x3")
    return out


def linear_forward(mod, x):
    if linear_xf32_ok(x, mod.weight):
        return linear_xf32(x, mod.weight, mod.bias)
    if gemm_x3_takes(x, mod.weight):
        return gemm_x3(x, mod.weight, mod.bias)
    return F.linear(x, mod.weight, mod.bias)


def install_linear_dispatch(module) -> int:
    n = 0
    for m in module.modules():
        if type(m) is torch.nn.Linear:
            m.forward = functools.partial(linear_forward, m)
            n += 1
    return n


WINO_FLOP_LOG = None


def _pack_wino_x3(weight):
    lib = _lib.load()
    co, ci = weight.shape[:2]
    packed = torch.empty(int(lib.tsplat_wino_weight_bf16x3_bytes(co, ci)), dtype=torch.uint8, device=weight.device)
    w = _f32(weight)
    _lib.check(lib.tsplat_wino_weight_bf16x3(_lib.ptr(w), _lib.ptr(packed), co, ci, _lib.stream_ptr(weight.device)),
               "tsplat_wino_weight_bf16x3")
    return packed


def wino_pack_weight_bf16x3(weight):
    return _derived(weight, "wino_x3", _pack_wino_x3)


_FEW = True
FEW_MIN_PX = 131072
FEW_MAX_CI = 64
FEW_MAX_CO = 32


def _few_ok(srcs, n: int, h: int, w: int, co: int, others=()) -> bool:
    ci = sum(t.shape[1] for t in srcs)
    return (_FEW and co <= FEW_MAX_CO and ci <= FEW_MAX_CI and n * h * w >= FEW_MIN_PX and w % 4 == 0
            and all(t.data_ptr() % 16 == 0 for t in (*srcs, *others) if t is not None)
            and int(_lib.load().tsplat_conv3x3_few_form(n, ci, h, w, co)) != 0)


def _int32_array(values):
    return ctypes.cast((ctypes.c_int32 * len(values))(*values), ctypes.c_void_p)


def _src_arrays(srcs):
    ptrs = (ctypes.c_void_p * len(srcs))(*[_lib.ptr(t) for t in srcs])
    return ctypes.cast(ptrs, ctypes.c_void_p), _int32_array([t.shape[1] for t in srcs])


def conv3x3_wino(x, weight, bias=None, act: str = "none", extra=(), precision: str | None = None, residual=None,
                 residual2=None, relu_in: bool = False):
    lib = _lib.load()
    precision = precision or _DENSE
    if precision != "bf16x3" and (relu_in or residual is not None or residual2 is not None):
        y = conv3x3_wino(torch.relu(x) if relu_in else x, weight, bias, act,
                         tuple(torch.relu(t) for t in extra) if relu_in else extra, precision)
        for r in (residual, residual2):
            if r is not None:
                y = y + r
        return y
    srcs = [_f32(t) for t in (x, *extra)]
    n, _, h, w = srcs[0].shape
    co = weight.shape[0]
    if WINO_FLOP_LOG is not None:
        ci = sum(t.shape[1] for t in srcs)
        WINO_FLOP_LOG.append((2.0 * 16 * ci * co * n * ((h + 1) // 2) * ((w + 1) // 2), _conv_flop(n * h * w, co, ci, 3)))
    y = torch.empty((n, co, h, w), dtype=torch.float32, device=x.device)
    pb = _f32(bias) if bias is not None else None
    ptrs, chans = _src_arrays(srcs)
    if precision == "bf16x3":
        res = [_f32(r) if r is not None else None for r in (residual, residual2)]
        for r in res:
            if r is not None and tuple(r.shape) != tuple(y.shape):
                raise ValueError(f"residual {tuple(r.shape)} != output {tuple(y.shape)}")
        if _few_ok(srcs, n, h, w, co, (y, *res)):
            rc = lib.tsplat_conv3x3_few_bf16x3_fwd(
                ptrs, chans, len(srcs), _lib.ptr(conv_pack_weight_x3(weight)), _lib.ptr(pb), _lib.ptr(res[0]),
                _lib.ptr(res[1]), _lib.ptr(y), n, h, w, co, _WINO_ACT[act], int(relu_in), _lib.stream_ptr(x.device))
            _lib.check(rc, "tsplat_conv3x3_few_bf16x3_fwd")
            return y
# ... 451 lines not shown
```

transplat_amd/model/depth_anything/dpt.py:

```python
from __future__ import annotations

import torch
import torch.nn.functional as F
from torch import nn


from ... import kernels
from .dinov2 import DINOv2



def _nchw3() -> bool:
    return kernels.split_mode()


def _resize(x, modifier: dict, align_corners: bool):
    if (align_corners and x.is_cuda and x.dtype == torch.bfloat16 and x.shape[1] % 4 == 0
            and torch.is_autocast_enabled("cuda") and x.is_contiguous(memory_format=torch.channels_last)):
        x = x.float().contiguous(memory_format=torch.channels_last)
    if (align_corners and x.is_cuda and x.dtype == torch.float32 and x.shape[1] % 4 == 0
            and x.is_contiguous(memory_format=torch.channels_last)):
        if "size" in modifier:
            size = modifier["size"]
        else:
            sf = modifier["scale_factor"]
            size = (int(x.shape[-2] * sf), int(x.shape[-1] * sf))
        return kernels.resize_bilinear_nhwc(x, size)
    if align_corners and x.is_cuda and x.dtype == torch.float32 and x.dim() == 4 and x.is_contiguous():
        if "size" in modifier:
            size = modifier["size"]
        else:
            sf = modifier["scale_factor"]
            size = (int(x.shape[-2] * sf), int(x.shape[-1] * sf))
        return kernels.interpolate_bilinear_ac(x, size)
    return F.interpolate(x, **modifier, mode="bilinear", align_corners=align_corners)


class ResidualConvUnit(nn.Module):
    def __init__(self, features, activation, bn):
        super().__init__()
        self.bn = bn
        self.conv1 = nn.Conv2d(features, features, kernel_size=3, stride=1, padding=1, bias=True)
        self.conv2 = nn.Conv2d(features, features, kernel_size=3, stride=1, padding=1, bias=True)
        if bn:
            self.bn1 = nn.BatchNorm2d(features)
            self.bn2 = nn.BatchNorm2d(features)
        self.activation = activation

    def _epilogue_ok(self, x) -> bool:
        return (not self.bn and isinstance(self.activation, nn.ReLU) and x.dtype == torch.float32
                and self.conv1.weight.dtype == torch.float32 and x.shape[1] % 4 == 0
                and not torch.is_autocast_enabled("cuda"))

    def forward(self, x, skip=None):
        if (_nchw3() and not self.bn and isinstance(self.activation, nn.ReLU) and x.is_cuda and x.is_contiguous()
                and kernels.conv_route(kernels.conv_module_call(self.conv1, (x,)), kernels.SITE_FORWARD) == "wino"
                and (skip is None or skip.is_contiguous())):
            out = kernels.conv3x3_wino(x, self.conv1.weight, self.conv1.bias, relu_in=True)
            return kernels.conv3x3_wino(out, self.conv2.weight, self.conv2.bias, relu_in=True, residual=x,
                                        residual2=skip)
        if self._epilogue_ok(x):
            out = kernels.conv_nhwc_epilogue(self.conv1, self.activation(x), "relu")
            return kernels.conv_nhwc_epilogue(self.conv2, out, "none", x, skip)
        out = self.conv1(self.activation(x))
        if self.bn:
            out = self.bn1(out)
        out = self.conv2(self.activation(out))
        if self.bn:
            out = self.bn2(out)
        return out + x if skip is None else skip + (out + x)


class FeatureFusionBlock(nn.Module):
    def __init__(self, features, activation, bn=False, align_corners=True, size=None):
        super().__init__()
        self.align_corners = align_corners
        self.out_conv = nn.Conv2d(features, features, kernel_size=1, stride=1, padding=0, bias=True)
        self.resConfUnit1 = ResidualConvUnit(features, activation, bn)
        self.resConfUnit2 = ResidualConvUnit(features, activation, bn)
        self.size = size

    def forward(self, *xs, size=None):
        output = xs[0]
        if len(xs) == 2:
            output = self.resConfUnit1(xs[1], skip=output)
        output = self.resConfUnit2(output)
        if size is None and self.size is None:
            modifier = {"scale_factor": 2}
        elif size is None:
            modifier = {"size": self.size}
        else:
            modifier = {"size": size}
        output = _resize(output, modifier, self.align_corners)
        return self.out_conv(output)


class _Scratch(nn.Module):
    pass


class DPTHead(nn.Module):
    def __init__(self, in_channels, features=256, use_bn=False, out_channels=(256, 512, 1024, 1024),
                 use_clstoken=False):
        super().__init__()
        if use_clstoken:
            raise NotImplementedError("Depth-Anything-V2 ViT-B runs without the class-token readout")
        self.use_clstoken = use_clstoken
        self.projects = nn.ModuleList([nn.Conv2d(in_channels, oc, kernel_size=1, stride=1, padding=0)
                                       for oc in out_channels])
        self.resize_layers = nn.ModuleList([
            nn.ConvTranspose2d(out_channels[0], out_channels[0], kernel_size=4, stride=4, padding=0),
            nn.ConvTranspose2d(out_channels[1], out_channels[1], kernel_size=2, stride=2, padding=0),
            nn.Identity(),
            nn.Conv2d(out_channels[3], out_channels[3], kernel_size=3, stride=2, padding=1)])
        s = _Scratch()
        s.layer1_rn = nn.Conv2d(out_channels[0], features, 3, 1, 1, bias=False)
        s.layer2_rn = nn.Conv2d(out_channels[1], features, 3, 1, 1, bias=False)
        s.layer3_rn = nn.Conv2d(out_channels[2], features, 3, 1, 1, bias=False)
        s.layer4_rn = nn.Conv2d(out_channels[3], features, 3, 1, 1, bias=False)
        s.stem_transpose = None
        act = nn.ReLU(False)
        s.refinenet1 = FeatureFusionBlock(features, act, bn=use_bn)
        s.refinenet2 = FeatureFusionBlock(features, act, bn=use_bn)
        s.refinenet3 = FeatureFusionBlock(features, act, bn=use_bn)
        s.refinenet4 = FeatureFusionBlock(features, act, bn=use_bn)
        s.output_conv1 = nn.Conv2d(features, features // 2, kernel_size=3, stride=1, padding=1)
        s.output_conv2 = nn.Sequential(
            nn.Conv2d(features // 2, 32, kernel_size=3, stride=1, padding=1), nn.ReLU(True),
            nn.Conv2d(32, 1, kernel_size=1, stride=1, padding=0), nn.ReLU(True), nn.Identity())
        self.scratch = s

    def _channels_last_weights(self):
        for m in self.modules():
            if isinstance(m, (nn.Conv2d, nn.ConvTranspose2d)) and m.weight.dim() == 4:
                m.weight.data = m.weight.data.contiguous(memory_format=torch.channels_last)
        self._cl_done = True

    def prepare(self, is_cuda: bool):
        if not getattr(self, "_cl_done", False) and is_cuda and not _nchw3():
            self._channels_last_weights()

    def reassemble(self, i, x, patch_h, patch_w):
        x = x.permute(0, 2, 1).reshape((x.shape[0], x.shape[-1], patch_h, patch_w))
        if _nchw3():
            x = self.resize_layers[i](self.projects[i](x.contiguous())).contiguous()
            return getattr(self.scratch, f"layer{i + 1}_rn")(x).contiguous()
        x = self.resize_layers[i](self.projects[i](x))
        return getattr(self.scratch, f"layer{i + 1}_rn")(x)

    def forward(self, out_features, patch_h, patch_w, raw_tail: bool = False):
        self.prepare(out_features[0][0].is_cuda)
        layer_1_rn, layer_2_rn, layer_3_rn, layer_4_rn = [self.reassemble(i, x[0], patch_h, patch_w)
                                                          for i, x in enumerate(out_features)]
        s = self.scratch
        path_4 = s.refinenet4(layer_4_rn, size=layer_3_rn.shape[2:])
        path_3 = s.refinenet3(path_4, layer_3_rn, size=layer_2_rn.shape[2:])
        path_2 = s.refinenet2(path_3, layer_2_rn, size=layer_1_rn.shape[2:])
        path_1 = s.refinenet1(path_2, layer_1_rn)
        final_out = s.output_conv1(path_1)
        out_feature = final_out.detach()
        final_out = _resize(final_out, {"size": (int(patch_h * 14), int(patch_w * 14))}, True)
        oc = s.output_conv2
        if (_nchw3() and final_out.is_contiguous()
                and kernels.conv_route(kernels.conv_module_call(oc[0], (final_out,)), kernels.SITE_FORWARD) == "wino"):
            h = kernels.conv3x3_wino(final_out, oc[0].weight, oc[0].bias, act="relu")
            if raw_tail and isinstance(oc[3], nn.ReLU) and isinstance(oc[4], nn.Identity):
                return oc[2](h), out_feature
            return oc[4](oc[3](oc[2](h))), out_feature
        if (final_out.dtype == torch.float32 and not torch.is_autocast_enabled("cuda")
                and final_out.is_cuda and final_out.is_contiguous(memory_format=torch.channels_last)):
            h = kernels.conv_nhwc_epilogue(oc[0], final_out, "relu")
            return oc[4](oc[3](oc[2](h))), out_feature
        return oc(final_out), out_feature


class DepthAnythingV2(nn.Module):
    def __init__(self, encoder="vitl", features=256, out_channels=(256, 512, 1024, 1024), use_bn=False,
                 use_clstoken=False):
        super().__init__()
        self.intermediate_layer_idx = {"vits": [2, 5, 8, 11], "vitb": [2, 5, 8, 11], "vitl": [4, 11, 17, 23]}
        self.encoder = encoder
        self.pretrained = DINOv2(model_name=encoder)
        self.depth_head = DPTHead(self.pretrained.embed_dim, features, use_bn, out_channels=out_channels,
                                  use_clstoken=use_clstoken)

    def forward(self, x, patches=None, raw_depth: bool = False):
        if patches is not None:
            pm, n_img, patch_h, patch_w = patches
            tokens = self.pretrained.prepare_tokens_patches(pm, n_img, patch_h, patch_w)
            is_cuda = True
        else:
            patch_h, patch_w = x.shape[-2] // 14, x.shape[-1] // 14
            tokens = None
            is_cuda = x.is_cuda
        head = self.depth_head
        head.prepare(is_cuda)
        from ...misc.benchmarker import stage

        with stage(None, "da_dinov2"):
            features = self.pretrained.get_intermediate_layers(x, self.intermediate_layer_idx[self.encoder],
                                                               return_class_token=True, tokens=tokens)
        with stage(None, "da_dpt"):
            depth, out_features = head(features, patch_h, patch_w, raw_tail=raw_depth)
        if raw_depth:
            return depth, out_features
        return F.relu(depth).squeeze(1), out_features
```

transplat_amd/model/encoder/encoder_trans.py:

```python
from __future__ import annotations

from contextlib import nullcontext
from dataclasses import dataclass, field
from typing import List, Literal, Optional

import torch
import torch.nn.functional as F
from einops import rearrange
from torch import nn

from ... import kernels, streams
from ...misc.benchmarker import stage
from ..depth_anything.dpt import DepthAnythingV2
from ..types import Gaussians
from .backbone.backbone_multiview import BackboneMultiview
from .common.gaussian_adapter import GaussianAdapter, GaussianAdapterCfg
from .encoder import Encoder
from .matching.depth_predictor_trans import DepthPredictorTrans

_DA_CONFIGS = {
    "vits": {"encoder": "vits", "features": 64, "out_channels": [48, 96, 192, 384]},
    "vitb": {"encoder": "vitb", "features": 128, "out_channels": [96, 192, 384, 768]},
    "vitl": {"encoder": "vitl", "features": 256, "out_channels": [256, 512, 1024, 1024]},
}


@dataclass
class OpacityMappingCfg:
    initial: float = 0.0
    final: float = 0.0
    warm_up: int = 1


@dataclass
class EncoderTransCfg:

    name: Literal["trans"] = "trans"
    d_feature: int = 128
    num_depth_candidates: int = 128
    num_surfaces: int = 1
    gaussian_adapter: GaussianAdapterCfg = field(default_factory=GaussianAdapterCfg)
    opacity_mapping: OpacityMappingCfg = field(default_factory=OpacityMappingCfg)
    gaussians_per_pixel: int = 1
    unimatch_weights_path: Optional[str] = None
    downscale_factor: int = 4
    shim_patch_size: int = 4
    multiview_trans_attn_split: int = 2
    costvolume_unet_feat_dim: int = 128
    costvolume_unet_channel_mult: List[int] = field(default_factory=lambda: [1, 1, 1])
    costvolume_unet_attn_res: List[int] = field(default_factory=lambda: [4])
    depth_unet_feat_dim: int = 32
    depth_unet_attn_res: List[int] = field(default_factory=lambda: [16])
    depth_unet_channel_mult: List[int] = field(default_factory=lambda: [1, 1, 1, 1, 1])
    wo_depth_refine: bool = False
    wo_cost_volume: bool = False
    wo_cost_volume_refine: bool = False
    num_context_views: int = 2
    da_encoder: str = "vitb"
    dense_dtype: str = "fp32"
    attn_dtype: str = "auto"


class EncoderTrans(Encoder[EncoderTransCfg]):
    def __init__(self, cfg: EncoderTransCfg) -> None:
        super().__init__(cfg)
        self.backbone = BackboneMultiview(feature_channels=cfg.d_feature, downscale_factor=cfg.downscale_factor)
        self.gaussian_adapter = GaussianAdapter(cfg.gaussian_adapter)
        da = _DA_CONFIGS[cfg.da_encoder]
        self.da_model = DepthAnythingV2(**da).eval()
        for p in self.da_model.parameters():
            p.requires_grad = False
        self.depth_predictor = DepthPredictorTrans(
            feature_channels=cfg.d_feature, upscale_factor=cfg.downscale_factor,
            num_depth_candidates=cfg.num_depth_candidates, costvolume_unet_feat_dim=cfg.costvolume_unet_feat_dim,
            costvolume_unet_channel_mult=tuple(cfg.costvolume_unet_channel_mult),
            costvolume_unet_attn_res=tuple(cfg.costvolume_unet_attn_res),
            gaussian_raw_channels=cfg.num_surfaces * (self.gaussian_adapter.d_in + 2),
            gaussians_per_pixel=cfg.gaussians_per_pixel, num_views=cfg.num_context_views,
            depth_unet_feat_dim=cfg.depth_unet_feat_dim, depth_unet_attn_res=cfg.depth_unet_attn_res,
            depth_unet_channel_mult=cfg.depth_unet_channel_mult, DA_size=da["features"] // 2)
        self.register_buffer("img_mean", torch.tensor([0.485, 0.456, 0.406]), persistent=False)
        self.register_buffer("img_std", torch.tensor([0.229, 0.224, 0.225]), persistent=False)
        kernels.install_conv2d_dispatch(self)
        kernels.install_linear_dispatch(self)

    def map_pdf_to_opacity(self, pdf, global_step: int):
        cfg = self.cfg.opacity_mapping
        x = cfg.initial + min(global_step / cfg.warm_up, 1) * (cfg.final - cfg.initial)
        exponent = 2**x
        return 0.5 * (1 - (1 - pdf) ** exponent + pdf ** (1 / exponent))

    def normalize_images(self, images):
        shape = [*[1] * (images.dim() - 3), 3, 1, 1]
        return (images - self.img_mean.reshape(*shape)) / self.img_std.reshape(*shape)

    def _dense(self):
        if self.cfg.dense_dtype == "bf16":
            return torch.autocast(device_type="cuda", dtype=torch.bfloat16)
        if self.cfg.dense_dtype == "bf16x3":
            return kernels.dense_precision("bf16x3")
        if self.cfg.dense_dtype != "fp32":
            raise ValueError(f"dense_dtype {self.cfg.dense_dtype!r}")
        return nullcontext()

    def forward(self, context: dict, global_step: int = 0, deterministic: bool = False,
                visualization_dump: Optional[dict] = None, scene_names=None, benchmarker=None,
                analyze_feature_depth: bool = False, enable_saes: bool = False, saes_config=None) -> Gaussians:
        device = context["image"].device
        b, v, _, h, w = context["image"].shape

        def bench(tag):
            return stage(benchmarker, tag)

        def prep_intrinsics(intrinsics, extrinsics):
            with bench("encoder_1_prep_intrinsics"):
                intr_curr = intrinsics[:, :, :3, :3].clone().detach()
                intr_curr[:, :, 0, :] *= float(w)
                intr_curr[:, :, 1, :] *= float(h)
                camk = torch.eye(4, device=device).view(1, 1, 4, 4).repeat(b, v, 1, 1).float()
                camk[:, :, :3, :3] = intr_curr
                return torch.matmul(extrinsics.clone().detach(), kernels.small_inverse(camk))

        def camera_consts(intrinsics, extrinsics, near, far):
            with bench("encoder_cameras"):
                f = self.cfg.downscale_factor
                dp = self.depth_predictor.camera_prep(intrinsics, extrinsics, near, far, h // f, w // f)
                ad = kernels.adapter_camera_consts(extrinsics, intrinsics, (h, w), self.gaussian_adapter.d_sh)
            return dp, ad

        def depth_anything(images):
            with bench("encoder_3_depth_anything"), torch.no_grad(), self._dense():
                dino = self.da_model.pretrained
                tail = kernels.split_mode() and images.is_cuda and images.dtype == torch.float32
                if kernels.split_mode() and dino.patches_ok(images):
                    g = 252 // dino.patch_size
                    pm = kernels.da_patches(images, self.img_mean, self.img_std, (g, g), dino.patch_size)
                    da_depth, out_feature = self.da_model(None, patches=(pm, b * v, g, g), raw_depth=tail)
                else:
                    da_images = self.normalize_images(images)
                    da_images = torch.cat((da_images[:, :, 2:3], da_images[:, :, 0:2]), dim=2)
                    da_images = da_images.reshape(b * v, 3, h, w)
                    da_images = kernels.interpolate_bilinear_ac(da_images, (252, 252))
                    da_depth, out_feature = self.da_model(da_images, raw_depth=tail)
                if tail:
                    da_depth = kernels.depth_norm(da_depth.float().reshape(b * v, *da_depth.shape[-2:]), (h, w))
                    return da_depth.view(b, v, 1, h, w), out_feature.float()
                da_depth = kernels.interpolate_bilinear_ac(da_depth[None].float().contiguous(), (h, w))
                da_depth = da_depth.view(b, v, 1, h, w).flatten(2)
                lo, hi = torch.aminmax(da_depth.view(b, v, h, w), dim=-1)
                da_min = lo.amin(dim=-1, keepdim=True)
                da_max = hi.amax(dim=-1, keepdim=True)
                da_depth = ((da_depth - da_min) / (da_max - da_min)).reshape(b, v, 1, h, w)
                return da_depth, out_feature.float()

        attn = self.cfg.attn_dtype
        if attn == "auto":
            attn = kernels.auto_attention(self.cfg.dense_dtype)

        def backbone(images, intrinsics, extrinsics, near, far):
            img2world = prep_intrinsics(intrinsics, extrinsics)
            with bench("encoder_2_backbone"), self._dense(), kernels.attention_precision(attn):
                tf, cf = self.backbone(images, attn_splits=self.cfg.multiview_trans_attn_split,
                                       return_cnn_features=True, img2world=img2world)
            return tf.float(), cf.float(), camera_consts(intrinsics, extrinsics, near, far)

        bb = streams.fork(device, backbone, context["image"], context["intrinsics"], context["extrinsics"],
                          context["near"], context["far"])
        da_depth, out_feature = depth_anything(context["image"])
        trans_features, cnn_features, (dp_cams, adapter_cams) = streams.join(bb)
        with bench("encoder_4_depth_predictor"), self._dense():
            begun = self.depth_predictor.begin(trans_features, context["intrinsics"], context["extrinsics"],
                                               context["near"], context["far"], cnn_features=cnn_features,
                                               benchmarker=benchmarker, cams=dp_cams)
        dino_feature = out_feature.view(b, v, *out_feature.shape[1:])

        extra_info = {"images": rearrange(context["image"], "b v c h w -> (v b) c h w"), "scene_names": scene_names}
        gpp = self.cfg.gaussians_per_pixel
        with bench("encoder_4_depth_predictor"), self._dense():
            depths, densities, raw_gaussians = self.depth_predictor(
                trans_features, context["intrinsics"], context["extrinsics"], context["near"], context["far"],
                gaussians_per_pixel=gpp, deterministic=deterministic, extra_info=extra_info,
                cnn_features=cnn_features, da_depth=da_depth, dino_feature=dino_feature, benchmarker=benchmarker,
                cams=dp_cams, begun=begun)
        depths, densities, raw_gaussians = depths.float(), densities.float(), raw_gaussians.float()

        with bench("encoder_5_gaussian_adapter"):
            srf = self.cfg.num_surfaces
            if srf != 1 or gpp != 1:
                raise NotImplementedError("TranSplat runs 1 surface and 1 Gaussian per pixel")
            x = self.cfg.opacity_mapping
            exponent = 2 ** (x.initial + min(global_step / x.warm_up, 1) * (x.final - x.initial))
            means, covariances, harmonics, opacities = self.gaussian_adapter(
                context["extrinsics"], context["intrinsics"], raw_gaussians, depths.reshape(b, v, h * w),
                densities.reshape(b, v, h * w), (h, w), opacity_exponent=exponent, gaussians_per_pixel=gpp,
                camera_consts=adapter_cams)
        if visualization_dump is not None:
            visualization_dump["depth"] = rearrange(depths, "b v (h w) srf s -> b v h w srf s", h=h, w=w)
        return Gaussians(means, covariances, harmonics, opacities)

    def get_data_shim(self):
        patch = self.cfg.shim_patch_size * self.cfg.downscale_factor

        def data_shim(batch):
            from ...dataset_shims import apply_patch_shim

            return apply_patch_shim(batch, patch_size=patch)

        return data_shim
```

transplat_amd/model/encoder/matching/depth_predictor_trans.py:

```python
from __future__ import annotations

import torch
import torch.nn.functional as F
from einops import rearrange, repeat
from torch import nn

from .... import kernels, streams
from ....misc.benchmarker import stage
from ...utils.cam_param_encoder import cam_param_encoder
from ...utils.uv_transformer import UVTransformer
from .ldm_unet import UNetModel, run_sequential


def _conv_upsample_gelu(seq: nn.Sequential, x):
    conv, up, act = seq
    if (not isinstance(act, nn.GELU) or act.approximate != "none" or up.mode != "bilinear"
            or not up.align_corners or float(up.scale_factor) != int(up.scale_factor)):
        return seq(x)
    call = kernels.conv_module_call(conv, (x,))
    y = kernels.conv_run(kernels.conv_route(call, kernels.SITE_HEAD, skip=("bf16",)), call, conv.weight, (x,))
    return kernels.upsample_bilinear_act(y, int(up.scale_factor), conv.bias, "gelu")


def _conv_gelu_conv(seq: nn.Sequential, x, extra=()):
    if not (len(seq) == 3 and isinstance(seq[1], nn.GELU) and seq[1].approximate == "none"):
        return seq(torch.cat([x, *extra], dim=1) if extra else x)
    return kernels.conv_bias_act(seq[2], kernels.conv_bias_act(seq[0], x, "gelu", extra=extra))


_GATE_AHEAD = True
_PACKED_AHEAD = True
_NO_ZERO_QUERY = True


@torch.autocast("cuda", enabled=False)
def camera_lists(intrinsics, extrinsics, near, far, num_samples: int, h: int, w: int):
    b, v = intrinsics.shape[:2]
    pose_curr_lists = []
    init_view_order = list(range(v))
    if v > 2:
        for idx in range(1, v):
            cur_view_order = init_view_order[idx:] + init_view_order[:idx]
            cur = [kernels.small_inverse(extrinsics[:, v1].clone().detach()) @ extrinsics[:, v0].clone().detach()
                   for v0, v1 in zip(init_view_order, cur_view_order)]
            pose_curr_lists.append(torch.cat(cur, dim=0))
    else:
        pose_ref = extrinsics[:, 0].clone().detach()
        pose_tgt = extrinsics[:, 1].clone().detach()
        pose = kernels.small_inverse(pose_tgt) @ pose_ref
        pose_curr_lists = [torch.cat((pose, kernels.small_inverse(pose)), dim=0)]
    intr_curr = intrinsics[:, :, :3, :3].clone().detach()
    intr_curr[:, :, 0, :] *= float(w)
    intr_curr[:, :, 1, :] *= float(h)
    intr_curr = rearrange(intr_curr, "b v ... -> (v b) ...", b=b, v=v)
    min_depth = rearrange(1.0 / far.clone().detach(), "b v -> (v b) 1")
    max_depth = rearrange(1.0 / near.clone().detach(), "b v -> (v b) 1")
    depth_candi_curr = (min_depth + torch.linspace(0.0, 1.0, num_samples, device=min_depth.device).unsqueeze(0)
                        * (max_depth - min_depth)).float()
    depth_candi_curr = repeat(depth_candi_curr, "vb d -> vb d () ()")
    return intr_curr, pose_curr_lists, depth_candi_curr


def match_img2world(intr_curr, extrinsics):
    b, v = extrinsics.shape[:2]
    with torch.autocast("cuda", enabled=False):
        camk = torch.eye(4, device=intr_curr.device).view(1, 4, 4).repeat(intr_curr.shape[0], 1, 1).float()
        camk[:, :3, :3] = intr_curr
        c2w = rearrange(extrinsics.clone().detach(), "b v ... -> (v b) ...", b=b, v=v)
        return torch.matmul(c2w, kernels.small_inverse(camk)).reshape(-1, 16)


def prepare_feat_proj_data_lists(features, intrinsics, extrinsics, near, far, num_samples, cams=None):
    b, v, _, h, w = features.shape
    feat_lists = [rearrange(features, "b v ... -> (v b) ...")]
    for idx in range(1, v):
        feat_lists.append(rearrange(torch.roll(features, -idx, dims=1), "b v ... -> (v b) ..."))
    if cams is None:
        cams = camera_lists(intrinsics, extrinsics, near, far, num_samples, h, w)
    intr_curr, pose_curr_lists, depth_candi_curr = cams
    return feat_lists, intr_curr, pose_curr_lists, depth_candi_curr.type_as(features)


_VIEW_PAIRS = {3: ((0, 1), (1, 2), (2, 0)), 4: ((0, 1), (1, 2), (2, 3), (3, 0), (0, 2), (1, 3))}


class DepthPredictorTrans(nn.Module):
    def __init__(self, feature_channels=128, upscale_factor=4, num_depth_candidates=32, costvolume_unet_feat_dim=128,
                 costvolume_unet_channel_mult=(1, 1, 1), costvolume_unet_attn_res=(), gaussian_raw_channels=-1,
                 gaussians_per_pixel=1, num_views=2, depth_unet_feat_dim=64, depth_unet_attn_res=(),
                 depth_unet_channel_mult=(1, 1, 1), DA_size=128, **kwargs):
        super().__init__()
        self.num_depth_candidates = num_depth_candidates
        self.regressor_feat_dim = costvolume_unet_feat_dim
        self.upscale_factor = upscale_factor
        input_channels = num_depth_candidates + feature_channels
        channels = self.regressor_feat_dim
        self.corr_refine_net = nn.Sequential(
            nn.Conv2d(input_channels, channels, 3, 1, 1), nn.GroupNorm(8, channels), nn.GELU(),
            UNetModel(image_size=None, in_channels=channels, model_channels=channels, out_channels=channels,
                      num_res_blocks=1, attention_resolutions=costvolume_unet_attn_res,
                      channel_mult=costvolume_unet_channel_mult, num_head_channels=32, dims=2, postnorm=True,
                      num_frames=num_views, use_cross_view_self_attn=True),
            nn.Conv2d(channels, num_depth_candidates, 3, 1, 1))
        self.regressor_residual = nn.Conv2d(input_channels, num_depth_candidates, 1, 1, 0)
        self.depth_head_lowres = nn.Sequential(
            nn.Conv2d(num_depth_candidates, num_depth_candidates * 2, 3, 1, 1), nn.GELU(),
            nn.Conv2d(num_depth_candidates * 2, num_depth_candidates, 3, 1, 1))
        proj_in_channels = feature_channels + feature_channels
        upsample_out_channels = feature_channels
        self.upsampler = nn.Sequential(
            nn.Conv2d(proj_in_channels, upsample_out_channels, 3, 1, 1),
            nn.Upsample(scale_factor=upscale_factor, mode="bilinear", align_corners=True), nn.GELU())
        self.proj_feature = nn.Conv2d(upsample_out_channels, depth_unet_feat_dim, 3, 1, 1)
        input_channels = 3 + 1 + depth_unet_feat_dim + 1 + 1
        channels = depth_unet_feat_dim
        self.refine_unet = nn.Sequential(
            nn.Conv2d(input_channels, channels, 3, 1, 1), nn.GroupNorm(4, channels), nn.GELU(),
            UNetModel(image_size=None, in_channels=channels, model_channels=channels, out_channels=channels,
                      num_res_blocks=1, attention_resolutions=depth_unet_attn_res,
                      channel_mult=depth_unet_channel_mult, num_head_channels=32, dims=2, postnorm=True,
                      num_frames=num_views, use_cross_view_self_attn=True))
        gau_in = depth_unet_feat_dim + 3 + feature_channels
        self.to_gaussians = nn.Sequential(
            nn.Conv2d(gau_in, gaussian_raw_channels * 2, 3, 1, 1), nn.GELU(),
            nn.Conv2d(gaussian_raw_channels * 2, gaussian_raw_channels, 3, 1, 1))
        channels = depth_unet_feat_dim
        self.to_disparity = nn.Sequential(
            nn.Conv2d(channels, channels * 2, 3, 1, 1), nn.GELU(),
            nn.Conv2d(channels * 2, gaussians_per_pixel * 2, 3, 1, 1))
        self.embed_dims = 128
        self.coarse_transformer = UVTransformer(embed_dims=self.embed_dims, mode="coarse", num_layers=1)
        self.fine_transformer = UVTransformer(embed_dims=self.embed_dims, mode="fine", num_layers=2)
        self.cam_param_encoder = cam_param_encoder(in_channels=DA_size, mid_channels=128, embed_dims=128)

    def camera_prep(self, intrinsics, extrinsics, near, far, h: int, w: int) -> dict:
        intr, poses, disp = camera_lists(intrinsics, extrinsics, near, far, self.num_depth_candidates, h, w)
        out = {"lists": (intr, poses, disp)}
        if intrinsics.shape[1] == 2:
            out["img2world"] = match_img2world(intr, extrinsics)
            gate = self.cam_param_encoder.gate(out["img2world"]) if _GATE_AHEAD else None
            if gate is not None:
                out["gate"] = gate
            if _PACKED_AHEAD and intr.is_cuda and intr.dtype == poses[0].dtype == torch.float32:
                out["packed"] = kernels.pack_cameras_fused(intr, poses[0])
        return out

    def coarse_two(self, intr_curr, pose_curr, disp_candi_curr, features, cams_packed=None):
        b, v, c, h, w = features.shape
        cameras = (intr_curr, pose_curr, disp_candi_curr.flatten(1).float())
        if cams_packed is not None:
            cameras += (cams_packed,)
        feat_cl = features.flatten(3).transpose(2, 3).contiguous()
        query = None if _NO_ZERO_QUERY else torch.zeros((b * v, h * w, self.embed_dims), device=features.device,
                                                        dtype=features.dtype)
        corr = self.coarse_transformer([features], query, w, h, cameras=cameras, channel_last=feat_cl)
        return corr, cameras, feat_cl

    def fine_two(self, coarse, intr_curr, extrinsics, dino_feature, features, img2world=None, gate=None):
        b, v, c, h, w = features.shape
        corr, cameras, feat_cl = coarse
        if img2world is None:
            img2world = match_img2world(intr_curr, extrinsics)
        pos_feature = self.cam_param_encoder(dino_feature, img2world, gate=gate, channel_last=b == 1)
        if pos_feature.dim() == 3:
            bev_pos = pos_feature
        else:
            bev_pos = rearrange(pos_feature, "(v b) c h w -> (b v) (h w) c", v=v, b=b).contiguous()
        corr = self.fine_transformer([features], corr, w, h, bev_pos=bev_pos, cameras=cameras, channel_last=feat_cl)
        return rearrange(corr, "(b v) (h w) c -> (v b) c h w", b=b, v=v, h=h, w=w)

    def match_two(self, intr_curr, pose_curr, extrinsics, disp_candi_curr, dino_feature, features, img2world=None):
        coarse = self.coarse_two(intr_curr, pose_curr, disp_candi_curr, features)
        return self.fine_two(coarse, intr_curr, extrinsics, dino_feature, features, img2world)

    def match_pairs(self, intr_curr, pose_curr_lists, extrinsics, disp_candi_curr, dino_feature, features):
        b, v = features.shape[:2]
        blk = lambda t, a: t[a * b:(a + 1) * b]
        parts = []
        for a, c in _VIEW_PAIRS[v]:
            pose = torch.cat((blk(pose_curr_lists[(c - a - 1) % v], a), blk(pose_curr_lists[(a - c - 1) % v], c)))
            pair = lambda t: torch.cat((blk(t, a), blk(t, c)))
            corr = self.match_two(pair(intr_curr), pose, torch.stack((extrinsics[:, a], extrinsics[:, c]), 1),
                                  pair(disp_candi_curr), pair(dino_feature),
                                  torch.stack((features[:, a], features[:, c]), 1))
            parts.append((corr[:b], corr[b:]))
        per_view = []
        for k in range(v):
            halves = [p[0] for (a, _), p in zip(_VIEW_PAIRS[v], parts) if a == k]
            halves += [p[1] for (_, c), p in zip(_VIEW_PAIRS[v], parts) if c == k]
            per_view.append(torch.stack(halves, dim=0).mean(dim=0))
        return torch.cat(per_view, dim=0)

    def _projection(self, feat01, cnn_features):
        proj_feat_in_fullres = _conv_upsample_gelu(self.upsampler, torch.cat((feat01, cnn_features), dim=1))
        return proj_feat_in_fullres, self.proj_feature(proj_feat_in_fullres)

    def begin(self, features, intrinsics, extrinsics, near, far, cnn_features=None, benchmarker=None, cams=None):
        b, v, c, h, w = features.shape

        with stage(benchmarker, "encoder_4a_prep_features"):
            if cnn_features is not None:
                cnn_features = rearrange(cnn_features, "b v ... -> (v b) ...")
            feat_comb_lists, intr_curr, pose_curr_lists, disp_candi_curr = prepare_feat_proj_data_lists(
                features, intrinsics, extrinsics, near, far, num_samples=self.num_depth_candidates,
                cams=cams["lists"] if cams is not None else None)
            feat01 = feat_comb_lists[0]
            proj = streams.fork(features.device, self._projection, feat01, cnn_features)
        coarse = None
        if v == 2:
            with stage(None, "dp_coarse"):
                coarse = self.coarse_two(intr_curr, pose_curr_lists[0], disp_candi_curr, features,
                                         cams.get("packed") if cams is not None else None)
        return {"lists": (intr_curr, pose_curr_lists, disp_candi_curr), "feat01": feat01, "proj": proj,
                "coarse": coarse}

    def forward(self, features, intrinsics, extrinsics, near, far, gaussians_per_pixel=1, deterministic=True,
                extra_info=None, cnn_features=None, da_depth=None, dino_feature=None, benchmarker=None, cams=None,
                begun=None):
        b, v, c, h, w = features.shape
        if begun is None:
            begun = self.begin(features, intrinsics, extrinsics, near, far, cnn_features, benchmarker, cams)
        intr_curr, pose_curr_lists, disp_candi_curr = begun["lists"]
        feat01, proj = begun["feat01"], begun["proj"]
        if da_depth is not None:
            da_depth = rearrange(da_depth, "b v ... -> (v b) ...")
        if dino_feature is not None:
            dino_feature = rearrange(dino_feature, "b v ... -> (v b) ...")
            dino_feature = kernels.interpolate_bilinear_ac(dino_feature, (h, w))
        with stage(benchmarker, "encoder_4b_cost_volume_matching"):
            img2world = cams.get("img2world") if cams is not None else None
            if begun["coarse"] is not None:
                gate = cams.get("gate") if cams is not None else None
                raw_correlation_in = torch.cat((self.fine_two(begun["coarse"], intr_curr, extrinsics, dino_feature,
                                                              features, img2world, gate), feat01), dim=1)
            else:
                raw_correlation_in = self._match(v, intr_curr, pose_curr_lists, extrinsics, disp_candi_curr,
                                                 dino_feature, features, feat01, img2world)
        with stage(benchmarker, "encoder_4c_cost_volume_unet"):
            raw_correlation = (run_sequential(self.corr_refine_net, raw_correlation_in)
                               + self.regressor_residual(raw_correlation_in))
        with stage(benchmarker, "encoder_4d_coarse_depth"):
            coarse_disps, pdf_max, fullres_disps = self._coarse_depth(raw_correlation, disp_candi_curr)
        with stage(benchmarker, "encoder_4e_depth_refine_unet"):
            proj_feat_in_fullres, proj_feature = streams.join(proj)
            refine_out = run_sequential(self.refine_unet, torch.cat(
                (extra_info["images"], da_depth, proj_feature, fullres_disps, pdf_max), dim=1))
        with stage(benchmarker, "encoder_4f_gaussian_head"):
            raw_gaussians = _conv_gelu_conv(self.to_gaussians, refine_out,
                                            extra=(extra_info["images"], proj_feat_in_fullres))
            raw_gaussians = rearrange(raw_gaussians, "(v b) c h w -> b v (h w) c", v=v, b=b)
            head = _conv_gelu_conv(self.to_disparity, refine_out)
            if gaussians_per_pixel == 1:
                depths, densities = kernels.depth_tail(fullres_disps, head, near, far)
                depths = depths.view(b, v, -1, 1, 1)
                densities = densities.view(b, v, -1, 1, 1)
            else:
                delta_disps, raw_densities = head.split(gaussians_per_pixel, dim=1)
                densities = repeat(F.sigmoid(raw_densities), "(v b) dpt h w -> b v (h w) srf dpt", b=b, v=v, srf=1)
                fine_disps = (fullres_disps + delta_disps).clamp(1.0 / rearrange(far, "b v -> (v b) () () ()"),
                                                                 1.0 / rearrange(near, "b v -> (v b) () () ()"))
                depths = repeat(1.0 / fine_disps, "(v b) dpt h w -> b v (h w) srf dpt", b=b, v=v, srf=1)
        return depths, densities, raw_gaussians

    def _match(self, v, intr_curr, pose_curr_lists, extrinsics, disp_candi_curr, dino_feature, features, feat01,
               img2world=None):
        if v == 2:
            raw_correlation_in = self.match_two(intr_curr, pose_curr_lists[0], extrinsics, disp_candi_curr,
                                                dino_feature, features, img2world)
        elif v in _VIEW_PAIRS:
            raw_correlation_in = self.match_pairs(intr_curr, pose_curr_lists, extrinsics, disp_candi_curr,
                                                  dino_feature, features)
        else:
            raise NotImplementedError(f"{v} context views (the reference handles 2, 3 and 4)")
        return torch.cat((raw_correlation_in, feat01), dim=1)

    def _coarse_depth(self, raw_correlation, disp_candi_curr):
        logits = _conv_gelu_conv(self.depth_head_lowres, raw_correlation)
        if logits.dtype == torch.float32:
            coarse_disps, pdf_max = kernels.depth_softmax(logits, disp_candi_curr)
        else:
            pdf = F.softmax(logits, dim=1)
            coarse_disps = (disp_candi_curr * pdf).sum(dim=1, keepdim=True)
            pdf_max = torch.max(pdf, dim=1, keepdim=True)[0]
        pdf_max = F.interpolate(pdf_max, scale_factor=self.upscale_factor)
        up = int(self.upscale_factor)
        fullres_disps = kernels.interpolate_bilinear_ac(coarse_disps, (coarse_disps.shape[-2] * up,
                                                                       coarse_disps.shape[-1] * up))
        return coarse_disps, pdf_max, fullres_disps
```

transplat_amd/routes.py:

```python
from __future__ import annotations

from collections import Counter
from contextlib import contextmanager

import torch
from torch.utils._python_dispatch import TorchDispatchMode

from . import _lib

_HIP = {
    "tsplat_win_attn_x3_partials_fwd": ("window attention", "bf16x3 (split-bf16 products, fp32 softmax)"),
    "tsplat_win_attn_x3_fwd": ("window attention", "bf16x3 (split-bf16 products, fp32 softmax)"),
    "tsplat_win_attn_bf16_shift_fwd": ("window attention", "bf16 MFMA, fp32 softmax"),
    "tsplat_win_attn_bf16_fwd": ("window attention", "bf16 MFMA, fp32 softmax"),
    "tsplat_win_attn_partials_fwd": ("window attention", "exact fp32"),
    "tsplat_win_attn_fwd": ("window attention", "exact fp32"),
    "tsplat_conv3x3_wino_bf16x3_fwd": ("3x3 convs (HIP Winograd)", "bf16x3"),
    "tsplat_conv3x3_wino_bf16x3_ex_fwd": ("3x3 convs (HIP Winograd)", "bf16x3"),
    "tsplat_conv3x3_wino_bf16x3_cat_fwd": ("3x3 convs (HIP Winograd)", "bf16x3"),
    "tsplat_conv3x3_wino_f32_fwd": ("3x3 convs (HIP Winograd)", "exact fp32"),
    "tsplat_conv3x3_wino_cat_f32_fwd": ("3x3 convs (HIP Winograd)", "exact fp32"),
    "tsplat_conv3x3_few_bf16x3_fwd": ("direct convs (HIP)", "bf16x3"),
    "tsplat_conv2d_bf16x3_fwd": ("direct convs (HIP)", "bf16x3"),
    "tsplat_conv1x1_bf16x3_scaled_fwd": ("direct convs (HIP)", "bf16x3"),
    "tsplat_conv2d_f32_fwd": ("direct convs (HIP)", "exact fp32"),
    "tsplat_conv2d_f32_zsplit_fwd": ("direct convs (HIP)", "exact fp32"),
    "tsplat_conv2d_f32_nhwc_fwd": ("direct convs (HIP)", "exact fp32"),
    "tsplat_conv2d_bf16_fwd": ("direct convs (HIP)", "bf16"),
    "tsplat_linear_f32_fwd": ("transformer linears (HIP)", None),
    "tsplat_linear_f32_split_x3_fwd": ("transformer linears (HIP)", None),
    "tsplat_linear_f32_attn_merge_fwd": ("transformer linears (HIP)", None),
    "tsplat_gemm_x3_fwd": ("GEMMs (HIP)", "bf16x3"),
    "tsplat_gemm_x3_cat_fwd": ("GEMMs (HIP)", "bf16x3"),
    "tsplat_mha_x3_fwd": ("DINOv2 attention (HIP)", "bf16x3"),
    "tsplat_mha_x3_presplit_fwd": ("DINOv2 attention (HIP)", "bf16x3"),
    "tsplat_mha_f32_fwd": ("DINOv2 attention (HIP)", "exact fp32"),
    "tsplat_mha_bias_f32_fwd": ("DINOv2 attention (HIP)", "exact fp32"),
    "tsplat_qkv_attention_cf_fwd": ("U-Net attention (HIP)", "exact fp32"),
    "tsplat_uv_coarse_fwd": ("correlation (HIP)", "fp32"),
    "tsplat_uv_cross_table_fwd": ("correlation (HIP)", "fp32"),
    "tsplat_uv_cross_fwd": ("correlation (HIP)", "fp32"),
    "tsplat_uv_cross_fused_fwd": ("correlation (HIP)", "bf16x3 products, fp32 gather"),
    "tsplat_uv_cross_fused_ld_fwd": ("correlation (HIP)", "bf16x3 products, fp32 gather"),
    "tsplat_cam_gate_fwd": ("camera prep (HIP)", "exact fp32"),
    "tsplat_pack_cameras_fwd": ("camera prep (HIP)", "exact fp32"),
    "tsplat_msda_fwd": ("correlation (HIP)", "fp32"),
    "tsplat_msda_raw_fwd": ("correlation (HIP)", "fp32"),
    "tsplat_ms_deform_attn_fwd": ("correlation (HIP)", "fp32"),
    "tsplat_group_norm_fwd": ("norms (HIP)", "fp32"),
    "tsplat_group_norm_cat_res_fwd": ("norms (HIP)", "fp32"),
    "tsplat_group_norm_bf16_fwd": ("norms (HIP)", "bf16 I/O, fp32 statistics"),
    "tsplat_layer_norm128_fwd": ("norms (HIP)", None),
    "tsplat_residual_ln_fwd": ("norms (HIP)", "fp32"),
    "tsplat_residual_ln_slabs_fwd": ("norms (HIP)", "fp32"),
    "tsplat_residual_ln_slabs_bcast_fwd": ("norms (HIP)", "fp32"),
    "tsplat_residual_ln_bf16_fwd": ("norms (HIP)", "bf16 I/O, fp32 statistics"),
    "tsplat_da_patches_fwd": ("Depth-Anything glue (HIP)", "fp32"),
    "tsplat_depth_norm_fwd": ("Depth-Anything glue (HIP)", "fp32"),
    "tsplat_gaussian_adapter_fwd": ("gaussian adapter (HIP)", "fp32"),
    "tsplat_sh_rotation_fwd": ("gaussian adapter (HIP)", "fp32"),
    "tsplat_raster_fwd": ("rasterizer (HIP)", "fp32"),
    "tsplat_raster_depth_fwd": ("rasterizer (HIP)", "fp32"),
}
_ORDER = ("window attention", "transformer linears (HIP)", "GEMMs (HIP)", "3x3 convs (HIP Winograd)", "direct convs (HIP)",
          "DINOv2 attention (HIP)", "U-Net attention (HIP)", "library GEMMs (hipBLASLt)", "library convs (MIOpen)",
          "camera prep (HIP)", "correlation (HIP)", "norms (HIP)", "Depth-Anything glue (HIP)", "gaussian adapter (HIP)", "rasterizer (HIP)")
_GEMMS = {"mm", "addmm", "bmm", "baddbmm", "addbmm", "_scaled_mm"}
_CONVS = {"convolution", "_convolution", "cudnn_convolution", "miopen_convolution", "convolution_overrideable",
          "conv2d", "conv_transpose2d", "miopen_convolution_transpose"}


class Routes:
    def __init__(self):
        self.calls: Counter = Counter()
        self.library: list = []

    def note(self, what: str, route: str | None = None) -> None:
        cat = _HIP.get(what)
        if cat is None:
            return
        self.calls[(cat[0], route or cat[1] or "?")] += 1

    def lib(self, op: str, arith: str, shapes) -> None:
        cat = "library GEMMs (hipBLASLt)" if op in _GEMMS else "library convs (MIOpen)"
        self.calls[(cat, arith)] += 1
        self.library.append((op, arith, shapes))

    def by_category(self) -> dict:
        out: dict = {}
        for (cat, arith), n in self.calls.items():
            out.setdefault(cat, Counter())[arith] += n
        return out

    def label(self) -> str:
        cats = self.by_category()
        parts = []
        for cat in _ORDER:
            if cat == "library convs (MIOpen)" and cat not in cats:
                parts.append("library convs (MIOpen): none")
                continue
            if cat not in cats:
                continue
            items = ", ".join(f"{a} x{n}" for a, n in sorted(cats[cat].items(), key=lambda kv: -kv[1]))
            parts.append(f"{cat}: {items}")
        return "; ".join(parts)


class _LibraryOps(TorchDispatchMode):
    def __init__(self, routes: Routes):
        super().__init__()
        self.routes = routes

    def __torch_dispatch__(self, func, types, args=(), kwargs=None):
        kwargs = kwargs or {}
        name = func.overloadpacket.__name__
        if name in _GEMMS or name in _CONVS:
            ts = [a for a in args if torch.is_tensor(a)]
            if ts and ts[0].is_cuda:
                dt = ts[-1].dtype if name in _GEMMS else ts[0].dtype
                if name in _GEMMS and dt == torch.float32:
                    arith = "xf32 (emulated, bf16 MFMA)" if torch.backends.cuda.matmul.allow_tf32 else "exact fp32"
                elif name in _GEMMS and dt == torch.bfloat16:
                    from . import kernels

                    arith = ("bf16x3 (split-bf16 K = 3k)" if kernels.split_mode()
                             and not torch.is_autocast_enabled("cuda") else "bf16")
                else:
                    arith = {torch.float32: "fp32", torch.bfloat16: "bf16", torch.float16: "fp16"}.get(dt, str(dt))
                shapes = [tuple(t.shape) for t in ts]
                if name in _CONVS and len(args) >= 7:
                    shapes.append((tuple(args[3]), tuple(args[4]), bool(args[6])))
                self.routes.lib(name, arith, shapes)
        return func(*args, **kwargs)


@contextmanager
def record():
    routes = Routes()
    prev = _lib.ROUTE_HOOK
    _lib.ROUTE_HOOK = routes.note
    try:
        with _LibraryOps(routes):
            yield routes
    finally:
        _lib.ROUTE_HOOK = prev
```

Before: 515.3 views/s.

## Add in-place strided 1x1 conv, fused pixel-shuffle epilogue, and deferred DA depth tail

Adds a bf16x3 1x1 conv variant that reads channel-last token rows directly through strides, skipping the permute-and-contiguous copy in the DPT reassemble projection. A second variant writes the transposed-conv (1x1 plus pixel shuffle) output straight into the shuffled layout from the epilogue, removing the separate pixel_shuffle pass. The Depth-Anything head's final tail and depth normalization are deferred and run on the forked projection stream inside the depth predictor, so they overlap with the correlation and coarse-depth work. This brings more template instantiations and more complex stream dependencies.

```diff
diff --git a/include/transplat_hip.h b/include/transplat_hip.h
--- a/include/transplat_hip.h
+++ b/include/transplat_hip.h
@@ -246,6 +246,10 @@
                                      const float* bias, float* y, int32_t batch, int32_t height, int32_t width,
                                      int32_t c_out, int32_t channel_last, int32_t ksplit, int32_t zsplit,
                                      float* partials, int32_t* counters, void* stream);
+int tsplat_conv1x1_bf16x3_inplace_fwd(const float* x, int32_t c_in, int32_t px_stride, int64_t img_stride,
+                                      const void* w_packed, const float* bias, float* y, int32_t batch,
+                                      int32_t height, int32_t width, int32_t c_out, int32_t shuffle, int32_t ksplit,
+                                      int32_t zsplit, float* partials, int32_t* counters, void* stream);
 
 size_t tsplat_wino_weight_floats(int32_t c_out, int32_t c_in);
 int tsplat_wino_weight_f32(const float* weight, float* w_packed, int32_t c_out, int32_t c_in, void* stream);
diff --git a/transplat_amd/_lib.py b/transplat_amd/_lib.py
--- a/transplat_amd/_lib.py
+++ b/transplat_amd/_lib.py
@@ -105,6 +105,8 @@
     "tsplat_conv2d_f32_zsplit_fwd": (ctypes.c_int, [_P, _I32, _P, _I32, _P, _P, _P] + [_I32] * 9 + [_P, _P, _P]),
     "tsplat_conv2d_bf16x3_fwd": (ctypes.c_int, [_P, _I32, _P, _I32, _P, _P, _P] + [_I32] * 9 + [_P, _P, _P]),
     "tsplat_conv1x1_bf16x3_scaled_fwd": (ctypes.c_int, [_P, _I32, _P, _P, _P, _P] + [_I32] * 7 + [_P, _P, _P]),
+    "tsplat_conv1x1_bf16x3_inplace_fwd": (ctypes.c_int, [_P, _I32, _I32, ctypes.c_int64, _P, _P, _P] + [_I32] * 7
+                                          + [_P, _P, _P]),
     "tsplat_resize_bilinear_nhwc_fwd": (ctypes.c_int, [_P, _P] + [_I32] * 6 + [_P]),
     "tsplat_resize_bilinear_nchw_fwd": (ctypes.c_int, [_P, _P] + [_I32] * 5 + [_P]),
     "tsplat_upsample_bilinear_act_fwd": (ctypes.c_int, [_P, _P, _P] + [_I32] * 6 + [_P]),
diff --git a/transplat_amd/csrc/conv.hip b/transplat_amd/csrc/conv.hip
--- a/transplat_amd/csrc/conv.hip
+++ b/transplat_amd/csrc/conv.hip
@@ -15,6 +15,9 @@
     const float* res;
     const float* scale;
     int cl_out;
+    int cl_px;
+    long long cl_img;
+    int shuf;
     float* y;
     float* part;
     int* cnt;
@@ -26,8 +29,10 @@
     int npx;
 };
 
-template <bool NHWC>
+enum { kNCHW = 0, kNHWC = 1, kShuffle = 2 };
+template <int OUT>
 __device__ __forceinline__ void tile_epilogue(const Args& p, const floatx16& acc, float* sred) {
+    constexpr bool NHWC = OUT == kNHWC;
     const int lane = threadIdx.x & 63, w = threadIdx.x >> 6, ksplit = blockDim.x >> 6;
     const int cot = blockIdx.y;
     const int hwo = p.hout * p.wout;
@@ -69,7 +74,12 @@
     const int nsum = p.zsplit > 1 ? 1 : ksplit;
     for (int idx = threadIdx.x; idx < 1024; idx += blockDim.x) {
         int r, l;
-        if (NHWC) {
+        if (OUT == kShuffle) {
+            const int kx = idx & (p.shuf - 1), pl = (idx / p.shuf) & 31;
+            const int col = idx / (32 * p.shuf) * p.shuf + kx;
+            r = ((col >> 3) << 2) | (col & 3);
+            l = ((col >> 2) & 1) * 32 + pl;
+        } else if (NHWC) {
             const int col = idx & 31, pl = idx >> 5;
             r = ((col >> 3) << 2) | (col & 3);
             l = ((col >> 2) & 1) * 32 + pl;
@@ -84,7 +94,12 @@
         if (co >= p.cout || q >= p.npx) continue;
         if (p.bias) s += p.bias[co];
         size_t o;
-        if (NHWC) {
+        if (OUT == kShuffle) {
+            const int k = p.shuf, kk = k * k;
+            const int qn = q / hwo, qp = q - qn * hwo, qy = qp / p.wout, qx = qp - qy * p.wout;
+            const int oc = co / kk, t = co - oc * kk, ky = t / k, kx = t - ky * k;
+            o = (((size_t)qn * (p.cout / kk) + oc) * (k * p.hout) + k * qy + ky) * (k * p.wout) + k * qx + kx;
+        } else if (NHWC) {
             o = (size_t)q * p.cout + co;
         } else {
             const int qn = q / hwo, qp = q - qn * hwo;
@@ -190,8 +205,9 @@
     tile_epilogue<NHWC>(p, acc, sred);
 }
 
-template <int KS, int S, int UP, int NB, bool SC = false>
+template <int KS, int S, int UP, int NB, bool SC = false, bool CL = false, bool SHUF = false>
 __global__ void __launch_bounds__(1024) conv_x3_kernel(Args p) {
+    static_assert(!(CL || SHUF) || (KS == 1 && S == 1 && UP == 0 && !SC), "in-place layouts: the plain 1x1 only");
     extern __shared__ float sred[];
     constexpr int T = KS * KS, PAD = KS / 2;
     const int lane = threadIdx.x & 63, w = threadIdx.x >> 6, ksplit = blockDim.x >> 6;
@@ -217,7 +233,7 @@
     const int units = ng * T;
     const int gw = blockIdx.z * ksplit + w, gstride = ksplit * p.zsplit;
     const int nu = units > gw ? (units - gw + gstride - 1) / gstride : 0;
-    const float* x1 = p.x1 + (size_t)nb * p.c1 * hwi;
+    const float* x1 = CL ? p.x1 + (size_t)nb * p.cl_img + (size_t)pix * p.cl_px : p.x1 + (size_t)nb * p.c1 * hwi;
     const float* x2 = p.x2 ? p.x2 + (size_t)nb * p.c2 * hwi : p.x1;
     const float* sc = SC && p.scale ? p.scale + (size_t)nb * ci : nullptr;
 
@@ -247,15 +263,25 @@
                     o = off[tt];
                     tv = (vmask >> tt) & 1;
                 }
-#pragma unroll
-            for (int j = 0; j < 8; ++j) {
-                const int ch = 16 * g + 8 * h + j;
-                const int cc = min(ch, ci - 1);
-                const float* src = cc < p.c1 ? x1 + (size_t)cc * hwi : x2 + (size_t)(cc - p.c1) * hwi;
-                float v = src[o];
-                if (SC && sc) v *= sc[cc];
+            if constexpr (CL) {
+                const int ch = 16 * g + 8 * h;
+                const float4* row = reinterpret_cast<const float4*>(x1 + min(ch, ci - 8));
+                const float4 v0 = row[0], v1 = row[1];
+                const float v[8] = {v0.x, v0.y, v0.z, v0.w, v1.x, v1.y, v1.z, v1.w};
                 const unsigned mb = (ok && tv && ch < ci) ? ~0u : 0u;
-                xv[k][j] = __uint_as_float(__float_as_uint(v) & mb);
+#pragma unroll
+                for (int j = 0; j < 8; ++j) xv[k][j] = __uint_as_float(__float_as_uint(v[j]) & mb);
+            } else {
+#pragma unroll
+                for (int j = 0; j < 8; ++j) {
+                    const int ch = 16 * g + 8 * h + j;
+                    const int cc = min(ch, ci - 1);
+                    const float* src = cc < p.c1 ? x1 + (size_t)cc * hwi : x2 + (size_t)(cc - p.c1) * hwi;
+                    float v = src[o];
+                    if (SC && sc) v *= sc[cc];
+                    const unsigned mb = (ok && tv && ch < ci) ? ~0u : 0u;
+                    xv[k][j] = __uint_as_float(__float_as_uint(v) & mb);
+                }
             }
         }
         __builtin_amdgcn_sched_barrier(0);
@@ -274,11 +300,11 @@
     }
     if constexpr (SC) {
         if (p.cl_out) {
-            tile_epilogue<true>(p, acc, sred);
+            tile_epilogue<kNHWC>(p, acc, sred);
             return;
         }
     }
-    tile_epilogue<false>(p, acc, sred);
+    tile_epilogue<SHUF ? kShuffle : kNCHW>(p, acc, sred);
 }
 
 }
@@ -409,11 +435,19 @@
     return TSPLAT_OK;
 }
 
+struct X3Form {
+    bool scaled = false;
+    const float* scale = nullptr;
+    int32_t cl_out = 0;
+    int32_t cl_px = 0;
+    int64_t cl_img = 0;
+    int32_t shuf = 0;
+};
+
 static int conv_x3_launch(const float* x1, int32_t c1, const float* x2, int32_t c2, const void* w_packed,
                           const float* bias, float* y, int32_t batch, int32_t height, int32_t width, int32_t c_out,
                           int32_t ksize, int32_t stride, int32_t upsample, int32_t ksplit, int32_t zsplit,
-                          float* partials, int32_t* counters, bool scaled, const float* scale, int32_t cl_out,
-                          void* stream_) {
+                          float* partials, int32_t* counters, const X3Form& form, void* stream_) {
     using namespace tsplat::conv;
     if (!x1 || !w_packed || !y || batch <= 0 || height <= 0 || width <= 0 || c_out <= 0) return TSPLAT_EINVAL;
     if (zsplit < 1 || zsplit > 64 || (zsplit > 1 && (!partials || !counters))) return TSPLAT_EINVAL;
@@ -431,8 +465,11 @@
     p.wp = (const float*)w_packed;
     p.bias = bias;
     p.y = y;
-    p.scale = scale;
-    p.cl_out = cl_out;
+    p.scale = form.scale;
+    p.cl_out = form.cl_out;
+    p.cl_px = form.cl_px;
+    p.cl_img = form.cl_img;
+    p.shuf = form.shuf;
     p.c1 = c1;
     p.c2 = c2;
     p.cout = c_out;
@@ -464,17 +501,23 @@
         else if (nb == 4) hipLaunchKernelGGL((conv_x3_kernel<KS, S, UP, 4>), grid, block, lds, stream, p); \
         else hipLaunchKernelGGL((conv_x3_kernel<KS, S, UP, 2>), grid, block, lds, stream, p);             \
     } while (0)
-    if (scaled) {
-        if (nb == 1) hipLaunchKernelGGL((conv_x3_kernel<1, 1, 0, 1, true>), grid, block, lds, stream, p);
-        else if (nb == 3) hipLaunchKernelGGL((conv_x3_kernel<1, 1, 0, 3, true>), grid, block, lds, stream, p);
-        else if (nb == 4) hipLaunchKernelGGL((conv_x3_kernel<1, 1, 0, 4, true>), grid, block, lds, stream, p);
-        else hipLaunchKernelGGL((conv_x3_kernel<1, 1, 0, 2, true>), grid, block, lds, stream, p);
-    } else if (ksize == 3 && stride == 1 && !upsample) TSPLAT_X3_LAUNCH(3, 1, 0);
+#define TSPLAT_X3_1X1(...)                                                                                     \
+    do {                                                                                                       \
+        if (nb == 1) hipLaunchKernelGGL((conv_x3_kernel<1, 1, 0, 1, __VA_ARGS__>), grid, block, lds, stream, p);     \
+        else if (nb == 3) hipLaunchKernelGGL((conv_x3_kernel<1, 1, 0, 3, __VA_ARGS__>), grid, block, lds, stream, p); \
+        else if (nb == 4) hipLaunchKernelGGL((conv_x3_kernel<1, 1, 0, 4, __VA_ARGS__>), grid, block, lds, stream, p); \
+        else hipLaunchKernelGGL((conv_x3_kernel<1, 1, 0, 2, __VA_ARGS__>), grid, block, lds, stream, p);             \
+    } while (0)
+    if (form.scaled) TSPLAT_X3_1X1(true);
+    else if (form.cl_px > 0) TSPLAT_X3_1X1(false, true, false);
+    else if (form.shuf > 0) TSPLAT_X3_1X1(false, false, true);
+    else if (ksize == 3 && stride == 1 && !upsample) TSPLAT_X3_LAUNCH(3, 1, 0);
     else if (ksize == 3 && stride == 2) TSPLAT_X3_LAUNCH(3, 2, 0);
     else if (ksize == 3) TSPLAT_X3_LAUNCH(3, 1, 1);
     else if (stride == 1) TSPLAT_X3_LAUNCH(1, 1, 0);
     else TSPLAT_X3_LAUNCH(1, 2, 0);
 #undef TSPLAT_X3_LAUNCH
+#undef TSPLAT_X3_1X1
     TSPLAT_PROF_END(tsplat::prof::kConv, stream);
     TSPLAT_CHECK_LAUNCH();
     return TSPLAT_OK;
@@ -486,7 +529,7 @@
                                         int32_t upsample, int32_t ksplit, int32_t zsplit, float* partials,
                                         int32_t* counters, void* stream_) {
     return conv_x3_launch(x1, c1, x2, c2, w_packed, bias, y, batch, height, width, c_out, ksize, stride, upsample,
-                          ksplit, zsplit, partials, counters, false, nullptr, 0, stream_);
+                          ksplit, zsplit, partials, counters, X3Form{}, stream_);
 }
 
 extern "C" int tsplat_conv1x1_bf16x3_scaled_fwd(const float* x, int32_t c_in, const float* scale, const void* w_packed,
@@ -494,6 +537,34 @@
                                                 int32_t width, int32_t c_out, int32_t channel_last, int32_t ksplit,
                                                 int32_t zsplit, float* partials, int32_t* counters, void* stream_) {
     if (channel_last != 0 && channel_last != 1) return TSPLAT_EINVAL;
+    X3Form form;
+    form.scaled = true;
+    form.scale = scale;
+    form.cl_out = channel_last;
     return conv_x3_launch(x, c_in, nullptr, 0, w_packed, bias, y, batch, height, width, c_out, 1, 1, 0, ksplit, zsplit,
-                          partials, counters, true, scale, channel_last, stream_);
-}
+                          partials, counters, form, stream_);
+}
+
+extern "C" int tsplat_conv1x1_bf16x3_inplace_fwd(const float* x, int32_t c_in, int32_t px_stride, int64_t img_stride,
+                                                 const void* w_packed, const float* bias, float* y, int32_t batch,
+                                                 int32_t height, int32_t width, int32_t c_out, int32_t shuffle,
+                                                 int32_t ksplit, int32_t zsplit, float* partials, int32_t* counters,
+                                                 void* stream_) {
+    X3Form form;
+    if ((px_stride > 0) == (shuffle > 0)) return TSPLAT_EINVAL;
+    if (px_stride > 0) {
+        if (c_in <= 0 || c_in % 8 || px_stride < c_in || px_stride % 4 || img_stride % 4 ||
+            img_stride < (int64_t)height * width * px_stride || reinterpret_cast<uintptr_t>(x) % 16)
+            return TSPLAT_EINVAL;
+        if ((int64_t)batch * img_stride >= (1ll << 31)) return TSPLAT_EINVAL;
+        form.cl_px = px_stride;
+        form.cl_img = img_stride;
+    } else {
+        if (px_stride != 0 || img_stride != 0 || !(shuffle == 2 || shuffle == 4) || c_out <= 0 ||
+            c_out % (shuffle * shuffle))
+            return TSPLAT_EINVAL;
+        form.shuf = shuffle;
+    }
+    return conv_x3_launch(x, c_in, nullptr, 0, w_packed, bias, y, batch, height, width, c_out, 1, 1, 0, ksplit, zsplit,
+                          partials, counters, form, stream_);
+}
diff --git a/transplat_amd/kernels.py b/transplat_amd/kernels.py
--- a/transplat_amd/kernels.py
+++ b/transplat_amd/kernels.py
@@ -901,6 +901,44 @@
     return y
 
 
+_ROWS_IN = True
+_SHUFFLE_OUT = True
+
+
+def _conv1x1_inplace(x, ci, px_stride, img_stride, weight, bias, n, h, w, shuffle, y):
+    lib = _lib.load()
+    co = weight.shape[0]
+    tiles = ((n * h * w + 31) // 32) * ((co + 31) // 32)
+    ksplit, z = _conv_x3_shape(tiles, (ci + 15) // 16)
+    part = cnt = None
+    if z > 1:
+        part = torch.empty(tiles * z * 1024, dtype=torch.float32, device=y.device)
+        cnt = _zsplit_counters(y.device, tiles)
+    pb = _f32(bias) if bias is not None else None
+    rc = lib.tsplat_conv1x1_bf16x3_inplace_fwd(_lib.ptr(x), ci, px_stride, img_stride,
+                                               _lib.ptr(conv_pack_weight_x3(weight)), _lib.ptr(pb), _lib.ptr(y), n, h, w,
+                                               co, shuffle, ksplit, z, _lib.ptr(part), _lib.ptr(cnt),
+                                               _lib.stream_ptr(y.device))
+    _lib.check(rc, "tsplat_conv1x1_bf16x3_inplace_fwd")
+    return y
+
+
+def conv1x1_rows(mod, rows, h: int, w: int):
+    n, hw, c = rows.shape
+    x = rows.permute(0, 2, 1).reshape(n, c, h, w)
+    if not (_ROWS_IN and split_mode() and rows.is_cuda and getattr(mod.forward, "func", None) is conv2d_forward
+            and mod.weight.dim() == 4 and hw == h * w and c % 8 == 0 and rows.stride(2) == 1
+            and rows.stride(1) % 4 == 0 and rows.stride(0) % 4 == 0 and rows.stride(1) >= c
+            and rows.stride(0) >= hw * rows.stride(1) and n * rows.stride(0) < 2 ** 31 and rows.data_ptr() % 16 == 0):
+        return mod(x.contiguous())
+    call = conv_module_call(mod, (x,))._replace(contiguous=True)
+    if not (call.k == 1 and call.stride == 1 and conv_route(call, SITE_FORWARD) == "direct"
+            and conv_x3_wins(call.npx, call.ci, call.co, 1)):
+        return mod(x.contiguous())
+    y = torch.empty((n, call.co, h, w), dtype=torch.float32, device=rows.device)
+    return _conv1x1_inplace(rows, c, rows.stride(1), rows.stride(0), mod.weight, mod.bias, n, h, w, 0, y)
+
+
 def conv2d_direct(x1, weight, bias=None, stride: int = 1, x2=None, upsample: bool = False):
     lib = _lib.load()
     n, c1, h, w = x1.shape
@@ -977,6 +1015,10 @@
     ci, co = weight.shape[:2]
     w1 = _derived(weight, "convT", lambda t: t.permute(1, 2, 3, 0).reshape(co * s * s, ci, 1, 1).contiguous())
     b1 = _derived(bias, "convT_b", lambda t: t.repeat_interleave(s * s).contiguous()) if bias is not None else None
+    n, _, h, w = x.shape
+    if _SHUFFLE_OUT and split_mode() and s in (2, 4) and x.is_cuda and x.dim() == 4 and x.numel() < 2 ** 31:
+        y = torch.empty((n, co, s * h, s * w), dtype=torch.float32, device=x.device)
+        return _conv1x1_inplace(_f32(x), ci, 0, 0, w1, b1, n, h, w, s, y)
     return F.pixel_shuffle(conv2d_direct(x, w1, b1, 1), s)
 
 
diff --git a/transplat_amd/model/depth_anything/dpt.py b/transplat_amd/model/depth_anything/dpt.py
--- a/transplat_amd/model/depth_anything/dpt.py
+++ b/transplat_amd/model/depth_anything/dpt.py
@@ -141,14 +141,14 @@
             self._channels_last_weights()
 
     def reassemble(self, i, x, patch_h, patch_w):
+        if _nchw3():
+            x = self.resize_layers[i](kernels.conv1x1_rows(self.projects[i], x, patch_h, patch_w)).contiguous()
+            return getattr(self.scratch, f"layer{i + 1}_rn")(x).contiguous()
         x = x.permute(0, 2, 1).reshape((x.shape[0], x.shape[-1], patch_h, patch_w))
-        if _nchw3():
-            x = self.resize_layers[i](self.projects[i](x.contiguous())).contiguous()
-            return getattr(self.scratch, f"layer{i + 1}_rn")(x).contiguous()
         x = self.resize_layers[i](self.projects[i](x))
         return getattr(self.scratch, f"layer{i + 1}_rn")(x)
 
-    def forward(self, out_features, patch_h, patch_w, raw_tail: bool = False):
+    def forward(self, out_features, patch_h, patch_w, raw_tail: bool = False, defer_tail: bool = False):
         self.prepare(out_features[0][0].is_cuda)
         layer_1_rn, layer_2_rn, layer_3_rn, layer_4_rn = [self.reassemble(i, x[0], patch_h, patch_w)
                                                           for i, x in enumerate(out_features)]
@@ -159,19 +159,24 @@
         path_1 = s.refinenet1(path_2, layer_1_rn)
         final_out = s.output_conv1(path_1)
         out_feature = final_out.detach()
+        if defer_tail:
+            return final_out, out_feature
+        return self.depth_tail(final_out, patch_h, patch_w, raw_tail), out_feature
+
+    def depth_tail(self, final_out, patch_h, patch_w, raw_tail: bool = False):
         final_out = _resize(final_out, {"size": (int(patch_h * 14), int(patch_w * 14))}, True)
-        oc = s.output_conv2
+        oc = self.scratch.output_conv2
         if (_nchw3() and final_out.is_contiguous()
                 and kernels.conv_route(kernels.conv_module_call(oc[0], (final_out,)), kernels.SITE_FORWARD) == "wino"):
             h = kernels.conv3x3_wino(final_out, oc[0].weight, oc[0].bias, act="relu")
             if raw_tail and isinstance(oc[3], nn.ReLU) and isinstance(oc[4], nn.Identity):
-                return oc[2](h), out_feature
-            return oc[4](oc[3](oc[2](h))), out_feature
+                return oc[2](h)
+            return oc[4](oc[3](oc[2](h)))
         if (final_out.dtype == torch.float32 and not torch.is_autocast_enabled("cuda")
                 and final_out.is_cuda and final_out.is_contiguous(memory_format=torch.channels_last)):
             h = kernels.conv_nhwc_epilogue(oc[0], final_out, "relu")
-            return oc[4](oc[3](oc[2](h))), out_feature
-        return oc(final_out), out_feature
+            return oc[4](oc[3](oc[2](h)))
+        return oc(final_out)
 
 
 class DepthAnythingV2(nn.Module):
@@ -184,7 +189,7 @@
         self.depth_head = DPTHead(self.pretrained.embed_dim, features, use_bn, out_channels=out_channels,
                                   use_clstoken=use_clstoken)
 
-    def forward(self, x, patches=None, raw_depth: bool = False):
+    def forward(self, x, patches=None, raw_depth: bool = False, defer_tail: bool = False):
         if patches is not None:
             pm, n_img, patch_h, patch_w = patches
             tokens = self.pretrained.prepare_tokens_patches(pm, n_img, patch_h, patch_w)
@@ -201,7 +206,11 @@
             features = self.pretrained.get_intermediate_layers(x, self.intermediate_layer_idx[self.encoder],
                                                                return_class_token=True, tokens=tokens)
         with stage(None, "da_dpt"):
-            depth, out_features = head(features, patch_h, patch_w, raw_tail=raw_depth)
+            depth, out_features = head(features, patch_h, patch_w, raw_tail=raw_depth, defer_tail=defer_tail)
+        if defer_tail:
+            if not raw_depth:
+                raise ValueError("defer_tail returns the raw depth's tail: raw_depth must be set")
+            return (lambda final_out: head.depth_tail(final_out, patch_h, patch_w, True), depth), out_features
         if raw_depth:
             return depth, out_features
         return F.relu(depth).squeeze(1), out_features
diff --git a/transplat_amd/model/encoder/encoder_trans.py b/transplat_amd/model/encoder/encoder_trans.py
--- a/transplat_amd/model/encoder/encoder_trans.py
+++ b/transplat_amd/model/encoder/encoder_trans.py
@@ -17,6 +17,8 @@
 from .common.gaussian_adapter import GaussianAdapter, GaussianAdapterCfg
 from .encoder import Encoder
 from .matching.depth_predictor_trans import DepthPredictorTrans
+
+_DEFER_DA_TAIL = True
 
 _DA_CONFIGS = {
     "vits": {"encoder": "vits", "features": 64, "out_channels": [48, 96, 192, 384]},
@@ -132,19 +134,33 @@
             with bench("encoder_3_depth_anything"), torch.no_grad(), self._dense():
                 dino = self.da_model.pretrained
                 tail = kernels.split_mode() and images.is_cuda and images.dtype == torch.float32
+                defer = _DEFER_DA_TAIL and tail and streams.enabled(images.device)
                 if kernels.split_mode() and dino.patches_ok(images):
                     g = 252 // dino.patch_size
                     pm = kernels.da_patches(images, self.img_mean, self.img_std, (g, g), dino.patch_size)
-                    da_depth, out_feature = self.da_model(None, patches=(pm, b * v, g, g), raw_depth=tail)
+                    da_depth, out_feature = self.da_model(None, patches=(pm, b * v, g, g), raw_depth=tail,
+                                                          defer_tail=defer)
                 else:
                     da_images = self.normalize_images(images)
                     da_images = torch.cat((da_images[:, :, 2:3], da_images[:, :, 0:2]), dim=2)
                     da_images = da_images.reshape(b * v, 3, h, w)
                     da_images = kernels.interpolate_bilinear_ac(da_images, (252, 252))
-                    da_depth, out_feature = self.da_model(da_images, raw_depth=tail)
+                    da_depth, out_feature = self.da_model(da_images, raw_depth=tail, defer_tail=defer)
+
+                def normalized(da_depth):
+                    da_depth = kernels.depth_norm(da_depth.float().reshape(b * v, *da_depth.shape[-2:]), (h, w))
+                    return da_depth.view(b, v, 1, h, w)
+
+                if defer:
+                    head_tail, final_out = da_depth
+
+                    def da_tail(final_out):
+                        with torch.no_grad(), self._dense():
+                            return normalized(head_tail(final_out))
+
+                    return (da_tail, final_out), out_feature.float()
                 if tail:
-                    da_depth = kernels.depth_norm(da_depth.float().reshape(b * v, *da_depth.shape[-2:]), (h, w))
-                    return da_depth.view(b, v, 1, h, w), out_feature.float()
+                    return normalized(da_depth), out_feature.float()
                 da_depth = kernels.interpolate_bilinear_ac(da_depth[None].float().contiguous(), (h, w))
                 da_depth = da_depth.view(b, v, 1, h, w).flatten(2)
                 lo, hi = torch.aminmax(da_depth.view(b, v, h, w), dim=-1)
@@ -167,11 +183,12 @@
         bb = streams.fork(device, backbone, context["image"], context["intrinsics"], context["extrinsics"],
                           context["near"], context["far"])
         da_depth, out_feature = depth_anything(context["image"])
+        da_tail, da_depth = (da_depth, None) if isinstance(da_depth, tuple) else (None, da_depth)
         trans_features, cnn_features, (dp_cams, adapter_cams) = streams.join(bb)
         with bench("encoder_4_depth_predictor"), self._dense():
             begun = self.depth_predictor.begin(trans_features, context["intrinsics"], context["extrinsics"],
                                                context["near"], context["far"], cnn_features=cnn_features,
-                                               benchmarker=benchmarker, cams=dp_cams)
+                                               benchmarker=benchmarker, cams=dp_cams, da_tail=da_tail)
         dino_feature = out_feature.view(b, v, *out_feature.shape[1:])
 
         extra_info = {"images": rearrange(context["image"], "b v c h w -> (v b) c h w"), "scene_names": scene_names}
diff --git a/transplat_amd/model/encoder/matching/depth_predictor_trans.py b/transplat_amd/model/encoder/matching/depth_predictor_trans.py
--- a/transplat_amd/model/encoder/matching/depth_predictor_trans.py
+++ b/transplat_amd/model/encoder/matching/depth_predictor_trans.py
@@ -195,7 +195,11 @@
         proj_feat_in_fullres = _conv_upsample_gelu(self.upsampler, torch.cat((feat01, cnn_features), dim=1))
         return proj_feat_in_fullres, self.proj_feature(proj_feat_in_fullres)
 
-    def begin(self, features, intrinsics, extrinsics, near, far, cnn_features=None, benchmarker=None, cams=None):
+    def _projection_da(self, feat01, cnn_features, da_fn, da_in):
+        return (*self._projection(feat01, cnn_features), da_fn(da_in))
+
+    def begin(self, features, intrinsics, extrinsics, near, far, cnn_features=None, benchmarker=None, cams=None,
+              da_tail=None):
         b, v, c, h, w = features.shape
 
         with stage(benchmarker, "encoder_4a_prep_features"):
@@ -205,7 +209,10 @@
                 features, intrinsics, extrinsics, near, far, num_samples=self.num_depth_candidates,
                 cams=cams["lists"] if cams is not None else None)
             feat01 = feat_comb_lists[0]
-            proj = streams.fork(features.device, self._projection, feat01, cnn_features)
+            if da_tail is not None:
+                proj = streams.fork(features.device, self._projection_da, feat01, cnn_features, *da_tail)
+            else:
+                proj = streams.fork(features.device, self._projection, feat01, cnn_features)
         coarse = None
         if v == 2:
             with stage(None, "dp_coarse"):
@@ -242,7 +249,9 @@
         with stage(benchmarker, "encoder_4d_coarse_depth"):
             coarse_disps, pdf_max, fullres_disps = self._coarse_depth(raw_correlation, disp_candi_curr)
         with stage(benchmarker, "encoder_4e_depth_refine_unet"):
-            proj_feat_in_fullres, proj_feature = streams.join(proj)
+            proj_feat_in_fullres, proj_feature, *deferred = streams.join(proj)
+            if deferred:
+                da_depth = rearrange(deferred[0], "b v ... -> (v b) ...")
             refine_out = run_sequential(self.refine_unet, torch.cat(
                 (extra_info["images"], da_depth, proj_feature, fullres_disps, pdf_max), dim=1))
         with stage(benchmarker, "encoder_4f_gaussian_head"):
diff --git a/transplat_amd/routes.py b/transplat_amd/routes.py
--- a/transplat_amd/routes.py
+++ b/transplat_amd/routes.py
@@ -23,6 +23,7 @@
     "tsplat_conv3x3_few_bf16x3_fwd": ("direct convs (HIP)", "bf16x3"),
     "tsplat_conv2d_bf16x3_fwd": ("direct convs (HIP)", "bf16x3"),
     "tsplat_conv1x1_bf16x3_scaled_fwd": ("direct convs (HIP)", "bf16x3"),
+    "tsplat_conv1x1_bf16x3_inplace_fwd": ("direct convs (HIP)", "bf16x3"),
     "tsplat_conv2d_f32_fwd": ("direct convs (HIP)", "exact fp32"),
     "tsplat_conv2d_f32_zsplit_fwd": ("direct convs (HIP)", "exact fp32"),
     "tsplat_conv2d_f32_nhwc_fwd": ("direct convs (HIP)", "exact fp32"),
```

Measured after the change: 522.1 views/s (median of 6 runs). +1.3%, better.
